# tupini07/StyleTransfer

Measured on AMD Instinct MI355X. Metric: Gatys iters/sec at 512×512 + fast_st images/sec at 256×256, 1/2/4/8 GPUs, higher is better.
Workload: dtype f32; 1 GPU; gatys_st 512x512 single image, Adam iterations (BASELINE configs[1]); one independent image per GPU (replicas); image=512, batch=1, parallelism=replicas1, graph=True

## Files before the change

### include/stx.h

```cpp
#ifndef STX_H_
#define STX_H_

#include <stddef.h>

#ifdef __cplusplus
extern "C" {
#endif

#define STX_AMAX_SLOTS 32

#define STX_OK 0
#define STX_E_INVALID 1001
#define STX_E_WORKSPACE 1002

#define STX_IN_RAW 0
#define STX_IN_RELU 1
#define STX_IN_RELU_POOL2 2
#define STX_IN_UPSAMPLE2 3
#define STX_IN_DILATE2 4

typedef struct stx_conv_params {
  const float* x;
  const float* wt;
  const float* bias;
// ... 34 lines not shown
  int unpool_out;
} stx_conv_params;

#define STX_GRAM_GROUP 8

int stx_version(void);
int stx_abi_layout(long long* out, int n);
const char* stx_last_error_string(void);
#define STX_ABI_VERSION 11
int stx_abi_version(void);

int stx_conv_weight_dims(int cin, int cout, int ks, int* cin_pad, int* cout_pad);

int stx_conv_weight_prep(const float* w, float* wt, int cout, int cin, int ks, int transpose,
                         void* stream);

size_t stx_conv_weight16_bytes(int cin, int cout, int ks, int transpose);
int stx_conv_weight_prep16(const float* w, void* wt16, float* w_amax, int cout, int cin, int ks,
                           int transpose, void* stream);
int stx_conv_weight_compose16(const float* A, int pitch, const float* a_amax, const float* w,
                              const float* w_amax, int cout, int cin, const float* scale,
                              void* wtT16, float* out_amax, void* stream);
int stx_conv_weight_prep16_pair(const float* w, void* wt16, void* wtT16, float* w_amax,
                                int cout, int cin, int ks, void* stream);
size_t stx_conv_weight16up_bytes(int cin, int cout);
int stx_conv_weight_prep16_up(const float* w, void* wt16_up, float* w_amax, int cout, int cin,
                              void* stream);
#define STX_WPREP_MAX 48
#define STX_WPREP_F32 0
#define STX_WPREP_F16 1
#define STX_WPREP_F16UP 2
typedef struct stx_wprep_job {
  const float* w;
  void* slab;
  float* w_amax;
  int kind, cout, cin, ks, transpose;
  int pad_;
} stx_wprep_job;
int stx_conv_weight_prep_batch(const stx_wprep_job* jobs, int njobs, void* stream);
int stx_amax(const float* x, long long n, float* out, void* stream);

int stx_conv_gram_tiles(const stx_conv_params* p);
int stx_conv_gram_groups(const stx_conv_params* p);

int stx_conv2d(const stx_conv_params* p, void* stream);

#define STX_WGRAD_NONE 0
#define STX_WGRAD_F32 1
#define STX_WGRAD_F16 2
#define STX_WGRAD_F16S2 3
#define STX_WGRAD_FEW16 4
typedef struct stx_wgrad_params {
  const float* x;
  const float* dy;
  float* dw;
  const float* x_amax;
  const float* dy_amax;
  void* ws;
  size_t ws_bytes;
  int accumulate;
  int n, cin, h, w, cout, ks, stride, pad, in_mode, ho, wo;
  int no_split;
} stx_wgrad_params;
int stx_conv2d_wgrad_plan(const stx_wgrad_params* p, size_t* ws_bytes);
int stx_conv2d_wgrad(const stx_wgrad_params* p, void* stream);
size_t stx_bias_grad_ws(int n, int c);
int stx_bias_grad(const float* dy, float* db, int n, int c, int hw, int accumulate,
                  void* ws, size_t ws_bytes, void* stream);

size_t stx_gram_ws(int b, int c, int hw);
int stx_gram(const float* z, float* g, int b, int c, int hw, float scale,
             const float* z_amax, void* ws, size_t ws_bytes, void* stream);

int stx_gram_coef_pitch(int c);
size_t stx_style_loss_parts(int b, int c, int hw, int* nparts);
typedef struct stx_loss_parts {
  const float* parts[8];
  int nparts[8];
  float inv[8];
  int k;
} stx_loss_parts;
int stx_loss_finalize(const stx_loss_parts* lp, float* losses, const float* extra, int m,
                      const float* w_host, float* total, void* stream);
int stx_gram_bwd(const float* coef, const float* z, float* dz, int b, int c, int h, int w,
                 const float* acc_scale_dev, const float* mask, const float* aux,
                 float aux_scale, int accumulate, void* stream);

#define STX_GUIDE_MAX 4
size_t stx_guided_style_ws(int b, int c, int hw, int R);
int stx_guided_style_loss(const float* z, const float* wts, float w_max, const float* target,
                          float* g_out, float* coef, float* loss_r, int b, int c, int hw, int R,
                          const float* lambda, float weight, const float* z_amax, void* ws,
                          size_t ws_bytes, void* stream);
int stx_guided_gram_bwd(const float* coef, const float* z, const float* wts, float* dz, int b,
                        int c, int h, int w, int R, const float* acc_scale_dev, int accumulate,
                        const float* z_amax, const float* coef_amax, void* stream);

size_t stx_color_stats_ws(int n, int h, int w);
int stx_color_stats(const float* x, double* stats, int n, int h, int w, void* ws,
                    size_t ws_bytes, void* stream);
int stx_color_affine(const float* x, const float* base, float* out, int n, int h, int w,
                     const float* M, const float* b, const float* lo, const float* hi,
                     void* stream);

size_t stx_mse_ws(long long n);
int stx_mse(const float* a, const float* b, long long n, int relu_inputs, int mode,
            float* out, float* grad, float gscale, void* ws, size_t ws_bytes, void* stream);
int stx_diff_scale(const float* a, const float* b, float* grad, long long n, float s0,
                   const float* s1_dev, const float* s2_dev, int relu, int accumulate,
                   void* stream);
#define STX_FIN_MAX 8
typedef struct stx_gram_fin_job {
  const float* parts;
  float* g_out;
  const float* target;
  float* coef;
  float* loss_parts;
  const float* mse_parts;
  float* mse_out;
  long long t_bstride;
  double mse_n;
  float scale, cA, alpha;
  int c, nsplit, b, cpad, mse_nparts;
  float* coef_amax;
} stx_gram_fin_job;
size_t stx_style_content_ws(int b, int c, int hw);
typedef struct stx_style_loss_params {
  const float* z;
  const float* parts;
  int nparts;
  const float* z_amax;
  const float* target;
  int target_batched;
  float* g_out;
  float* coef;
  float* loss;
  int b, c, hw;
  float weight, diag_alpha;
  const float* content;
  const float* mse_parts;
  float* mse_out;
  void* ws;
  size_t ws_bytes;
  stx_gram_fin_job* defer;
} stx_style_loss_params;
int stx_style_loss(const stx_style_loss_params* p, void* stream);
int stx_gram_finalize_batch(const stx_gram_fin_job* jobs, int njobs, void* stream);

int stx_loss_combine(const float* s, int k, const float* w_host, float* out, void* stream);

size_t stx_vec_ws(void);
int stx_vec_reduce(const float* a, const float* b, long long n, int op, float* out,
                   const float* mul, const float* add, float sgn, void* ws, size_t ws_bytes,
                   void* stream);
int stx_vec_axpby(float* y, const float* x, long long n, float a, const float* a_dev,
                  float a_sgn, float b, void* stream);
int stx_scalar_op(float* s, int op, int i, int j, int k, void* stream);

size_t stx_lbfgs_state_bytes(int m);
size_t stx_lbfgs_hist_bytes(long long n, int m);
size_t stx_lbfgs_ws(long long n, int m);
int stx_lbfgs_direction(float* x, const float* g, float* prev_g, float* hist, long long n, int m,
                        float lr, float tol_change, void* state, float* scal, void* ws,
                        size_t ws_bytes, void* stream);
int stx_lbfgs_grad_stats(const float* g, long long n, const float* loss, float* scal, float* clear,
                         int clear_n, void* ws, size_t ws_bytes, void* stream);

int stx_maxpool2x2_fwd(const float* x, float* y, long long* idx, int nc, int h, int w,
                       int relu_input, void* stream);
int stx_maxpool2x2_bwd(const float* dy, const long long* idx, float* dx, int nc, int h, int w,
                       void* stream);
int stx_relupool_bwd(const float* dp, const float* z, float* dz, int nc, int h, int w,
                     void* stream);
int stx_relu_fwd(const float* x, float* y, long long n, void* stream);
int stx_relu_bwd(const float* dy, const float* y, float* dx, long long n, void* stream);

size_t stx_adam_ws(void);
int stx_adam_step(float* p, const float* g, float* m, float* v, long long n, float lr,
                  float beta1, float beta2, float eps, int* step_dev, void* ws, void* stream);
int stx_adam_step_clear(float* p, const float* g, float* m, float* v, long long n, float lr,
                        float beta1, float beta2, float eps, int* step_dev, void* ws,
                        float* clear, int clear_n, void* stream);

int stx_instnorm_fwd(const float* x, const float* res, const float* gamma, const float* beta,
                     float* y, float* mean, float* rstd, int n, int c, int hw, float eps,
                     int relu, float* out_amax, void* stream);
size_t stx_instnorm_bwd_ws(int n, int c);
#define STX_PGRAD_MAX 32
typedef struct stx_in_pgrad_job {
  const float* parts;
  float* dgamma;
  float* dbeta;
  float* dbias_in;
  int n, c, accumulate, pad_;
} stx_in_pgrad_job;
int stx_instnorm_param_grads(const stx_in_pgrad_job* jobs, int njobs, void* stream);
int stx_instnorm_bwd(const float* dy, const float* beta, const float* x, const float* res,
                     const float* gamma, const float* mean, const float* rstd, float* du,
                     float* dgamma, float* dbeta, float* dbias_in, int n, int c, int hw, int relu,
                     int accumulate_params, float* out_amax, void* ws, size_t ws_bytes,
                     void* stream);

#define STX_CIN_MAX 32
typedef struct stx_cin_job {
  const float* gtab;
  const float* btab;
  float* gamma_n;
  float* beta_n;
  const float* parts;
  float* dgtab;
  float* dbtab;
  float* dbias_in;
  int c, accumulate;
} stx_cin_job;
int stx_cin_mix(const stx_cin_job* jobs, int njobs, const float* mix, int n, int S,
                void* stream);
int stx_cin_param_grads(const stx_cin_job* jobs, int njobs, const float* mix, int n, int S,
                        void* stream);

int stx_upsample2x_fwd(const float* x, float* y, int nc, int h, int w, void* stream);
int stx_upsample2x_bwd(const float* dy, float* dx, int nc, int h, int w, void* stream);

size_t stx_tv_ws(int n, int c, int h, int w);
int stx_tv_loss(const float* y, float* loss, float* grad, float gscale, const float* gscale_dev,
                int n, int c, int h, int w, float factor, void* ws, size_t ws_bytes,
                void* stream);

size_t stx_temporal_loss_ws(void);
int stx_temporal_loss(const float* y, const float* y_old, const float* x, const float* x_old,
                      long long n, float weight, float* out, void* ws, size_t ws_bytes,
                      void* stream);
int stx_temporal_loss_bwd(const float* y, const float* y_old, long long n, const float* fwd,
                          float weight, const float* g_dev, float* grad, int accumulate,
                          void* stream);

int stx_flow_compose(const float* const* prev, const float* const* fwd,
                     const float* const* bwd, int count, const float* fill, float* ref,
                     float* cmask, float* init, unsigned char* which, int n, int c, int h, int w,
                     void* stream);
int stx_flow_warp(const float* src, const float* flow, const float* fill, float* out,
                  float* valid, int n, int c, int h, int w, void* stream);
int stx_flow_consistency(const float* fwd, const float* bwd, float* cmask, int n, int h, int w,
                         void* stream);
size_t stx_masked_mse_ws(void);
int stx_masked_mse(const float* x, const float* ref, const float* mask, int n, int c, int hw,
                   float weight, float* out, float* add_to, float* grad, int accumulate,
                   void* ws, size_t ws_bytes, void* stream);

typedef struct {
  long long offset;
  int h, w;
  int top, left;
  int y0, y1;
  int resize_w, resize_h;
  int xcoef, ycoef;
  int xk, yk;
  long long tmp_offset;
} stx_image_meta;
int stx_resample_coeffs(int in_size, int out_size, int* bounds, int* kk, int kk_stride);
int stx_image_condition(const void* src, const stx_image_meta* meta, int b, int max_rows,
                        const int* coef, int size, const float* mean, const float* std_,
                        float* out, void* tmp, size_t tmp_bytes, void* stream);

#define STX_JPEG_OK 0
#define STX_JPEG_UNSUPPORTED 1
// ... 78 lines not shown
```

### styletransfer_amd/_native.py

```python
from __future__ import annotations

import ctypes as C
import os
import threading

_HERE = os.path.dirname(os.path.abspath(__file__))
LIB_PATH = os.environ.get("STX_LIB", os.path.join(_HERE, "libstx.so"))

STX_IN_RAW, STX_IN_RELU, STX_IN_RELU_POOL2, STX_IN_UPSAMPLE2, STX_IN_DILATE2 = range(5)
STX_AMAX_SLOTS = 32
STX_GRAM_GROUP = 8
STX_FLOW_JACOBI_MAXFUSE = 8
STX_ABI_VERSION = 11


def knob(name: str, default: str) -> str:
    if os.environ.get("STX_AB") != "1":
        return default
    return os.environ.get(name, default)

vp = C.c_void_p
i32 = C.c_int
i64 = C.c_longlong
f32 = C.c_float
# ... 34 lines not shown
class PGradJob(C.Structure):
    _fields_ = [("parts", vp), ("dgamma", vp), ("dbeta", vp), ("dbias_in", vp), ("n", i32),
                ("c", i32), ("accumulate", i32), ("pad_", i32)]


STX_PGRAD_MAX = 32


class CinJob(C.Structure):
    _fields_ = [("gtab", vp), ("btab", vp), ("gamma_n", vp), ("beta_n", vp), ("parts", vp),
                ("dgtab", vp), ("dbtab", vp), ("dbias_in", vp), ("c", i32), ("accumulate", i32)]


STX_CIN_MAX = 32


class LossParts(C.Structure):
    _fields_ = [("parts", vp * 8), ("nparts", i32 * 8), ("inv", f32 * 8), ("k", i32)]


class GramFinJob(C.Structure):
    _fields_ = [("parts", vp), ("g_out", vp), ("target", vp), ("coef", vp), ("loss_parts", vp),
                ("mse_parts", vp), ("mse_out", vp), ("t_bstride", i64), ("mse_n", C.c_double),
                ("scale", f32), ("cA", f32), ("alpha", f32), ("c", i32), ("nsplit", i32),
                ("b", i32), ("cpad", i32), ("mse_nparts", i32), ("coef_amax", vp)]


class StyleLossParams(C.Structure):
    _fields_ = [("z", vp), ("parts", vp), ("nparts", i32), ("z_amax", vp), ("target", vp),
                ("target_batched", i32), ("g_out", vp), ("coef", vp), ("loss", vp), ("b", i32),
                ("c", i32), ("hw", i32), ("weight", f32), ("diag_alpha", f32), ("content", vp),
                ("mse_parts", vp), ("mse_out", vp), ("ws", vp), ("ws_bytes", sz),
                ("defer", C.POINTER(GramFinJob))]


class WgradParams(C.Structure):
    _fields_ = [("x", vp), ("dy", vp), ("dw", vp), ("x_amax", vp), ("dy_amax", vp), ("ws", vp),
                ("ws_bytes", sz), ("accumulate", i32), ("n", i32), ("cin", i32), ("h", i32),
                ("w", i32), ("cout", i32), ("ks", i32), ("stride", i32), ("pad", i32),
                ("in_mode", i32), ("ho", i32), ("wo", i32), ("no_split", i32)]


class JpegDesc(C.Structure):
    _fields_ = [("status", i32), ("h", i32), ("w", i32), ("ncomp", i32), ("hs", i32 * 3),
                ("vs", i32 * 3), ("bw", i32 * 3), ("bh", i32 * 3), ("restart_interval", i32),
                ("coef_bytes", i64)]


class JpegJob(C.Structure):
    _fields_ = [("rgb_offset", i64), ("coef_offset", i64), ("qtab_offset", i64),
                ("tmp_offset", i64), ("h", i32), ("w", i32), ("ncomp", i32), ("raw", i32),
                ("hmax", i32), ("vmax", i32), ("bw", i32 * 3), ("bh", i32 * 3)]


class JpegEncJob(C.Structure):
    _fields_ = [("src_offset", i64), ("coef_offset", i64), ("qtab_offset", i64),
                ("tmp_offset", i64), ("h", i32), ("w", i32), ("ncomp", i32), ("fp32", i32),
                ("hmax", i32), ("vmax", i32), ("bw", i32 * 3), ("bh", i32 * 3),
                ("mean", f32 * 3), ("std_", f32 * 3)]


STX_JPEG_CHUNK = 32
STX_WGRAD_NONE, STX_WGRAD_F32, STX_WGRAD_F16, STX_WGRAD_F16S2, STX_WGRAD_FEW16 = range(5)
STX_FIN_MAX = 8
STX_GUIDE_MAX = 4


SIGNATURES = {
    "stx_version": (i32, []),
    "stx_abi_layout": (i32, [vp, i32]),
    "stx_last_error_string": (C.c_char_p, []),
    "stx_abi_version": (i32, []),
    "stx_conv_weight_dims": (i32, [i32, i32, i32, C.POINTER(i32), C.POINTER(i32)]),
    "stx_conv_weight_prep": (i32, [vp, vp, i32, i32, i32, i32, vp]),
    "stx_conv2d": (i32, [C.POINTER(ConvParams), vp]),
    "stx_conv_gram_tiles": (i32, [C.POINTER(ConvParams)]),
    "stx_conv_gram_groups": (i32, [C.POINTER(ConvParams)]),
    "stx_conv_weight16_bytes": (sz, [i32, i32, i32, i32]),
    "stx_conv_weight_prep16": (i32, [vp, vp, vp, i32, i32, i32, i32, vp]),
    "stx_conv_weight_prep16_pair": (i32, [vp, vp, vp, vp, i32, i32, i32, vp]),
    "stx_conv_weight16up_bytes": (sz, [i32, i32]),
    "stx_conv_weight_prep16_up": (i32, [vp, vp, vp, i32, i32, vp]),
    "stx_conv_weight_compose16": (i32, [vp, i32, vp, vp, vp, i32, i32, vp, vp, vp, vp]),
    "stx_amax": (i32, [vp, i64, vp, vp]),
    "stx_conv_weight_prep_batch": (i32, [C.POINTER(WprepJob), i32, vp]),
    "stx_conv2d_wgrad_plan": (i32, [C.POINTER(WgradParams), C.POINTER(sz)]),
    "stx_conv2d_wgrad": (i32, [C.POINTER(WgradParams), vp]),
    "stx_vec_ws": (sz, []),
    "stx_vec_reduce": (i32, [vp, vp, i64, i32, vp, vp, vp, f32, vp, sz, vp]),
    "stx_vec_axpby": (i32, [vp, vp, i64, f32, vp, f32, f32, vp]),
    "stx_scalar_op": (i32, [vp, i32, i32, i32, i32, vp]),
    "stx_lbfgs_state_bytes": (sz, [i32]),
    "stx_lbfgs_hist_bytes": (sz, [i64, i32]),
    "stx_lbfgs_ws": (sz, [i64, i32]),
    "stx_lbfgs_direction": (i32, [vp, vp, vp, vp, i64, i32, f32, f32, vp, vp, vp, sz, vp]),
    "stx_lbfgs_grad_stats": (i32, [vp, i64, vp, vp, vp, i32, vp, sz, vp]),
    "stx_bias_grad_ws": (sz, [i32, i32]),
    "stx_bias_grad": (i32, [vp, vp, i32, i32, i32, i32, vp, sz, vp]),
    "stx_gram_ws": (sz, [i32, i32, i32]),
    "stx_gram": (i32, [vp, vp, i32, i32, i32, f32, vp, vp, sz, vp]),
    "stx_gram_coef_pitch": (i32, [i32]),
    "stx_style_loss": (i32, [C.POINTER(StyleLossParams), vp]),
    "stx_style_content_ws": (sz, [i32, i32, i32]),
    "stx_gram_finalize_batch": (i32, [C.POINTER(GramFinJob), i32, vp]),
    "stx_gram_bwd": (i32, [vp, vp, vp, i32, i32, i32, i32, vp, vp, vp, f32, i32, vp]),
    "stx_guided_style_ws": (sz, [i32, i32, i32, i32]),
    "stx_guided_style_loss": (i32, [vp, vp, f32, vp, vp, vp, vp, i32, i32, i32, i32,
                                    C.POINTER(f32), f32, vp, vp, sz, vp]),
    "stx_guided_gram_bwd": (i32, [vp, vp, vp, vp, i32, i32, i32, i32, i32, vp, i32, vp, vp,
                                  vp]),
    "stx_color_stats_ws": (sz, [i32, i32, i32]),
    "stx_color_stats": (i32, [vp, vp, i32, i32, i32, vp, sz, vp]),
    "stx_color_affine": (i32, [vp, vp, vp, i32, i32, i32, C.POINTER(f32), C.POINTER(f32),
                               C.POINTER(f32), C.POINTER(f32), vp]),
    "stx_mse_ws": (sz, [i64]),
    "stx_mse": (i32, [vp, vp, i64, i32, i32, vp, vp, f32, vp, sz, vp]),
    "stx_diff_scale": (i32, [vp, vp, vp, i64, f32, vp, vp, i32, i32, vp]),
    "stx_loss_combine": (i32, [vp, i32, C.POINTER(f32), vp, vp]),
    "stx_style_loss_parts": (sz, [i32, i32, i32, C.POINTER(i32)]),
    "stx_loss_finalize": (i32, [C.POINTER(LossParts), vp, vp, i32, C.POINTER(f32), vp, vp]),
    "stx_maxpool2x2_fwd": (i32, [vp, vp, vp, i32, i32, i32, i32, vp]),
    "stx_maxpool2x2_bwd": (i32, [vp, vp, vp, i32, i32, i32, vp]),
    "stx_relupool_bwd": (i32, [vp, vp, vp, i32, i32, i32, vp]),
    "stx_relu_fwd": (i32, [vp, vp, i64, vp]),
    "stx_relu_bwd": (i32, [vp, vp, vp, i64, vp]),
    "stx_adam_ws": (sz, []),
    "stx_adam_step": (i32, [vp, vp, vp, vp, i64, f32, f32, f32, f32, vp, vp, vp]),
    "stx_adam_step_clear": (i32, [vp, vp, vp, vp, i64, f32, f32, f32, f32, vp, vp, vp, i32, vp]),
    "stx_instnorm_fwd": (i32, [vp, vp, vp, vp, vp, vp, vp, i32, i32, i32, f32, i32, vp, vp]),
    "stx_instnorm_bwd_ws": (sz, [i32, i32]),
    "stx_instnorm_param_grads": (i32, [C.POINTER(PGradJob), i32, vp]),
    "stx_instnorm_bwd": (i32, [vp, vp, vp, vp, vp, vp, vp, vp, vp, vp, vp, i32, i32, i32,
                               i32, i32, vp, vp, sz, vp]),
    "stx_cin_mix": (i32, [C.POINTER(CinJob), i32, vp, i32, i32, vp]),
    "stx_cin_param_grads": (i32, [C.POINTER(CinJob), i32, vp, i32, i32, vp]),
    "stx_upsample2x_fwd": (i32, [vp, vp, i32, i32, i32, vp]),
    "stx_upsample2x_bwd": (i32, [vp, vp, i32, i32, i32, vp]),
    "stx_tv_ws": (sz, [i32, i32, i32, i32]),
    "stx_tv_loss": (i32, [vp, vp, vp, f32, vp, i32, i32, i32, i32, f32, vp, sz, vp]),
    "stx_resample_coeffs": (i32, [i32, i32, vp, vp, i32]),
    "stx_image_condition": (i32, [vp, vp, i32, i32, vp, i32, vp, vp, vp, vp, sz, vp]),
    "stx_jpeg_info": (i32, [vp, sz, C.POINTER(JpegDesc)]),
    "stx_jpeg_entropy_decode": (i32, [vp, sz, vp, sz, vp]),
    "stx_jpeg_decode_batch": (i32, [C.POINTER(JpegJob), i32, vp, vp, vp, sz, vp]),
    "stx_jpeg_layout": (i32, [vp, i32]),
    "stx_jpeg_quant_tables": (i32, [i32, vp]),
    "stx_jpeg_encode_bound": (sz, [i32, i32, i32, i32, i32]),
    "stx_jpeg_entropy_encode": (i32, [vp, sz, i32, i32, i32, i32, i32, vp, vp, sz,
                                      C.POINTER(sz)]),
    "stx_jpeg_encode_batch": (i32, [C.POINTER(JpegEncJob), i32, vp, vp, vp, sz, vp]),
    "stx_jpeg_enc_layout": (i32, [vp, i32]),
    "stx_resample_plan": (i32, [i32, i32, i32, vp, vp, vp, i32]),
    "stx_resample2d_ws": (sz, [i32, i32, i32, i32, i32]),
    "stx_resample2d": (i32, [vp, vp, i32, i32, i32, i32, i32, vp, vp, vp, i32, vp, vp, vp, i32,
                             vp, sz, vp]),
    "stx_temporal_loss_ws": (sz, []),
    "stx_temporal_loss": (i32, [vp, vp, vp, vp, i64, f32, vp, vp, sz, vp]),
    "stx_temporal_loss_bwd": (i32, [vp, vp, i64, vp, f32, vp, vp, i32, vp]),
    "stx_flow_warp": (i32, [vp, vp, vp, vp, vp, i32, i32, i32, i32, vp]),
    "stx_flow_consistency": (i32, [vp, vp, vp, i32, i32, i32, vp]),
    "stx_flow_compose": (i32, [vp, vp, vp, i32, vp, vp, vp, vp, vp, i32, i32, i32, i32, vp]),
    "stx_masked_mse_ws": (sz, []),
    "stx_masked_mse": (i32, [vp, vp, vp, i32, i32, i32, f32, vp, vp, vp, i32, vp, sz, vp]),
    "stx_flow_pyramid": (i32, [i32, i32, i32, vp, vp, i32]),
    "stx_flow_luma": (i32, [vp, vp, i32, i32, i32, vp, vp, vp]),
    "stx_flow_linearize": (i32, [vp, vp, vp, vp, i32, i32, i32, vp]),
    "stx_flow_jacobi_ws": (sz, [i32, i32, i32]),
    "stx_flow_jacobi": (i32, [vp, vp, vp, i32, i32, i32, f32, i32, i32, vp, sz, vp]),
    "stx_flow_scale": (i32, [vp, i32, i32, i32, f32, f32, vp]),
}

_lib = None
_lock = threading.Lock()


class NativeError(RuntimeError):
    pass


def lib():
    global _lib
    if _lib is not None:
        return _lib
    with _lock:
        if _lib is None:
            if not os.path.exists(LIB_PATH):
                raise NativeError(
                    f"libstx.so not found at {LIB_PATH}; build it with "
                    f"`python -c 'import __graft_entry__ as g; g.build()'` "
                    f"(make -C styletransfer_amd/csrc)")
            try:
                L = C.CDLL(LIB_PATH)
            except OSError as e:
                raise NativeError(f"failed to load {LIB_PATH}: {e}") from e
            abi = L.stx_abi_version() if hasattr(L, "stx_abi_version") else None
            if abi != STX_ABI_VERSION:
                raise NativeError(f"{LIB_PATH}: ABI revision {abi}, this binding needs "
                                  f"{STX_ABI_VERSION} (include/stx.h STX_ABI_VERSION)")
            partial = os.environ.get("STX_LIB_PARTIAL") == "1"
            for name, (res, args) in SIGNATURES.items():
                if partial and not hasattr(L, name):
                    continue
                fn = getattr(L, name)
                fn.restype = res
                fn.argtypes = args
            _lib = L
    return _lib


def check(rc: int, what: str = ""):
    if rc != 0:
# ... 3 lines not shown
```

### styletransfer_amd/csrc/conv16.hip

```cpp
#include <stdlib.h>
#include <type_traits>

#include "common.h"
#include "conv_epi.h"
#include "wprep.h"
#include "../../include/stx.h"

namespace stx {

typedef _Float16 f16x8 __attribute__((ext_vector_type(8)));


template <int TW>
__device__ __forceinline__ void phase2_f16(f32x16 (&acc)[2][2], const stx_conv_params& p, int n,
                                           int co0, int ty0, int tx0, int wave, int h, int l32,
                                           char* smem) {
  constexpr int NPIX = 256, BM = 64;
  constexpr bool RP = TW == 64;
  const int tid = threadIdx.x;
  const size_t plane = (size_t)p.ho * p.wo;
  const float* __restrict__ A = p.p2_wt + (size_t)n * p.p2_wt_batch_stride;
  const int C2 = p.p2_c;
  const float s2 = p.p2_scale ? *p.p2_scale : 1.f;
  char* lz = smem;
  char* la = smem + 4 * NPIX * 16;
  const int q = tid & 63, cq = tid >> 6;
  const int qp = 4 * q, qrow = qp / TW, qcol = qp - qrow * TW;
  const int qy = ty0 + qrow, qx = tx0 + qcol;
  const bool vec = (p.wo & 3) == 0;
  const uint32_t zq_off = (qy < p.ho && qx < p.wo) ? (uint32_t)(qy * p.wo + qx) * 4u : BUF_OOB;
  const uint32_t pb = (uint32_t)plane * 4u;
  const float* __restrict__ z2 = p.p2_z + (size_t)n * C2 * plane;
  int bpix[2];
#pragma unroll
  for (int j = 0; j < 2; ++j) {
    int ty, tx;
    tile_pix<TW, RP>(wave, j, l32, ty, tx);
    bpix[j] = ty * TW + tx;
  }
  const int acg = tid >> 6, aco = tid & 63;
  struct Stage {
    f32x4 z[4];
    float a[8];
  };
  auto fetch = [&](int c0, Stage& g) {
    const auto rz = make_srd(z2 + (size_t)c0 * plane, (uint32_t)max(0, C2 - c0) * pb);
#pragma unroll
    for (int e = 0; e < 4; ++e) {
      const uint32_t o = zq_off + (uint32_t)(4 * cq + e) * pb;
      if (vec) {
        g.z[e] = buf_ld4(rz, o);
      } else {
#pragma unroll
        for (int k = 0; k < 4; ++k)
          g.z[e][k] = (qx + k < p.wo) ? buf_ld(rz, o + 4u * k) : 0.f;
      }
    }
    if (tid < 128) {
#pragma unroll
      for (int e = 0; e < 8; ++e) {
        const int c = c0 + acg * 8 + e, co = co0 + aco;
        g.a[e] = (c < C2 && co < p.cout_pad) ? A[(size_t)c * p.cout_pad + co] : 0.f;
      }
    }
  };
  Stage s0, s1;
  fetch(0, s0);
  if (16 < C2) fetch(16, s1);
  float m = 0.f;
  for (int base = 0; base < C2 * (BM / 4); base += 1024) {
    f32x4 v[4];
#pragma unroll
    for (int u = 0; u < 4; ++u) {
      const int idx = base + tid + 256 * u;
      const int c = idx / (BM / 4), q4 = idx - c * (BM / 4);
      const int co = co0 + 4 * q4;
      const f32x4 zero = {0.f, 0.f, 0.f, 0.f};
      v[u] = (c < C2 && co < p.cout_pad)
                 ? *reinterpret_cast<const f32x4*>(A + (size_t)c * p.cout_pad + co)
                 : zero;
    }
#pragma unroll
    for (int u = 0; u < 4; ++u)
#pragma unroll
      for (int e = 0; e < 4; ++e) m = fmaxf(m, fabsf(v[u][e]));
  }
  __shared__ float red2[4];
// ... 1306 lines not shown
    upd(v[3]);
  }
  for (long long i = 4 * n4 + t0; i < n; i += stride) upd(x[i]);
  block_max_to(out, m);
}

__device__ __forceinline__ void amax_slot_body(const float* __restrict__ x, long long n,
                                               float* __restrict__ out, int slot) {
  __shared__ float red[16];
  const long long n4 = n >> 2;
  const long long per = (n4 + STX_AMAX_SLOTS - 1) / STX_AMAX_SLOTS;
  const long long b0 = slot * per, b1 = min(n4, b0 + per);
  float m = 0.f;
  auto upd = [&](float v) {
    m = max_nan_wins(m, fabsf(v));
  };
#pragma unroll 4
  for (long long i = b0 + threadIdx.x; i < b1; i += 1024) {
    const f32x4 v = reinterpret_cast<const f32x4*>(x)[i];
    upd(v[0]);
    upd(v[1]);
    upd(v[2]);
    upd(v[3]);
  }
  if (slot == 0)
    for (long long i = 4 * n4 + threadIdx.x; i < n; i += 1024) upd(x[i]);
#pragma unroll
  for (int o = 32; o > 0; o >>= 1) {
    m = max_nan_wins(m, __shfl_xor(m, o, 64));
  }
  if ((threadIdx.x & 63) == 0) red[threadIdx.x >> 6] = m;
  __syncthreads();
  if (threadIdx.x == 0) {
    float r = red[0];
#pragma unroll
    for (int i = 1; i < 16; ++i) r = max_nan_wins(r, red[i]);
    out[slot] = r;
  }
}

__global__ void __launch_bounds__(1024) amax_slots_kernel(const float* __restrict__ x,
                                                          long long n, float* __restrict__ out) {
  amax_slot_body(x, n, out, blockIdx.x);
}

struct WprepAmax {
  const float* w[STX_WPREP_MAX];
  float* out[STX_WPREP_MAX];
  long long n[STX_WPREP_MAX];
};

__global__ void __launch_bounds__(1024) amax_batch_kernel(WprepAmax a) {
  const int j = blockIdx.x / STX_AMAX_SLOTS;
  amax_slot_body(a.w[j], a.n[j], a.out[j], blockIdx.x % STX_AMAX_SLOTS);
}

struct WprepJobs {
  stx_wprep_job job[STX_WPREP_MAX];
  int blk0[STX_WPREP_MAX + 1];
  int gin[STX_WPREP_MAX], gout[STX_WPREP_MAX];
  int njobs;
};

__global__ void __launch_bounds__(256) weight_prep_batch_kernel(WprepJobs b) {
  int j = 0;
  while (j + 1 < b.njobs && (int)blockIdx.x >= b.blk0[j + 1]) ++j;
  const stx_wprep_job& t = b.job[j];
  const int nb = b.blk0[j + 1] - b.blk0[j];
  const long long i0 = (long long)(blockIdx.x - b.blk0[j]) * 256 + threadIdx.x;
  const long long step = (long long)nb * 256;
  if (t.kind == STX_WPREP_F16)
    weight_prep16_body(t.w, reinterpret_cast<_Float16*>(t.slab), t.w_amax, t.cout, t.cin,
                       t.transpose, b.gin[j], b.gout[j], i0, step);
  else if (t.kind == STX_WPREP_F16UP)
    weight_prep16up_body(t.w, reinterpret_cast<_Float16*>(t.slab), t.w_amax, t.cout, t.cin,
                         b.gin[j] / 16, b.gout[j], i0, step);
  else
    weight_prep32_body(t.w, reinterpret_cast<float*>(t.slab), t.cout, t.cin, t.ks, t.transpose,
                       b.gin[j], b.gout[j], i0, step);
}

constexpr int WC_R = 16, WC_K = 64;

__global__ void __launch_bounds__(256)
weight_compose16_kernel(const float* __restrict__ A, int pitch, const float* __restrict__ a_amax,
                        const float* __restrict__ W, const float* __restrict__ w_amax, int C,
                        int cin, const float* __restrict__ scale, _Float16* __restrict__ slab,
                        float* __restrict__ out_amax) {
  typedef _Float16 f16x4 __attribute__((ext_vector_type(4)));
  const int K = cin * 9;
  __shared__ __attribute__((aligned(16))) float la[256][WC_R];
  __shared__ __attribute__((aligned(16))) float lw[256][WC_K];
  float (*red)[WC_R * WC_K] = reinterpret_cast<float (*)[WC_R * WC_K]>(&lw[0][0]);
  const int tid = threadIdx.x, lane = tid & 63, wave = tid >> 6;
  const int c0 = blockIdx.y * WC_R, k0 = blockIdx.x * WC_K;
  const float sc = scale ? *scale : 1.f;
  const float bound = fabsf(sc) * (float)C * read_amax(a_amax) * read_amax(w_amax);
  if (blockIdx.x == 0 && blockIdx.y == 0 && tid < STX_AMAX_SLOTS) out_amax[tid] = bound;
  const float sw = __builtin_ldexpf(1.f, 15 - amax_exp(bound));
  {
    constexpr int NLD = 256 * WC_K / 4 / 256;
    const auto ra = make_srd(A, (uint32_t)C * (uint32_t)pitch * 4u);
    const auto rw = make_srd(W, (uint32_t)C * (uint32_t)K * 4u);
    float av[WC_R];
#pragma unroll
    for (int r = 0; r < WC_R; ++r)
      av[r] = buf_ld(ra, (c0 + r < C && tid < C) ? (uint32_t)((c0 + r) * pitch + tid) * 4u : BUF_OOB);
    f32x4 v[NLD];
#pragma unroll
    for (int u = 0; u < NLD; ++u) {
      const int f = tid + 256 * u, co = f >> 4, k = k0 + 4 * (f & 15);
      v[u] = buf_ld4(rw, co < C && k < K ? (uint32_t)(co * K + k) * 4u : BUF_OOB);
    }
#pragma unroll
    for (int r = 0; r < WC_R; r += 4)
      *reinterpret_cast<f32x4*>(&la[tid][r]) = f32x4{av[r], av[r + 1], av[r + 2], av[r + 3]};
#pragma unroll
    for (int u = 0; u < NLD; ++u) {
      const int f = tid + 256 * u;
      *reinterpret_cast<f32x4*>(&lw[f >> 4][4 * (f & 15)]) = v[u];
    }
  }
  __syncthreads();
  const int r4 = 4 * (lane >> 4), q4 = 4 * (lane & 15);
  const int kk = k0 + q4;
  float acc[4][4];
#pragma unroll
  for (int a = 0; a < 4; ++a)
#pragma unroll
    for (int b = 0; b < 4; ++b) acc[a][b] = 0.f;
  const int cb = 64 * wave, ce = min(C, cb + 64);
#pragma unroll 8
  for (int co = cb; co < ce; ++co) {
    const f32x4 a4 = *reinterpret_cast<const f32x4*>(&la[co][r4]);
    const f32x4 w4 = *reinterpret_cast<const f32x4*>(&lw[co][q4]);
#pragma unroll
    for (int a = 0; a < 4; ++a)
#pragma unroll
      for (int b = 0; b < 4; ++b) acc[a][b] = fmaf(a4[a], w4[b], acc[a][b]);
  }
  __syncthreads();
  if (wave > 0) {
#pragma unroll
    for (int a = 0; a < 4; ++a)
#pragma unroll
      for (int b = 0; b < 4; ++b) red[wave - 1][(r4 + a) * WC_K + q4 + b] = acc[a][b];
  }
  __syncthreads();
  if (wave != 0) return;
  const int gout64 = rup(cin, 64);
  const int c = c0 + r4, chunk = c >> 4, cg = (c >> 3) & 1, e0 = c & 7;
#pragma unroll
  for (int b = 0; b < 4; ++b) {
    const int k = kk + b;
    if (k >= K || c >= C) continue;
    const int ci = k / 9, tap = k - 9 * ci, tapf = 8 - tap;
    f16x4 hi, lo;
#pragma unroll
    for (int a = 0; a < 4; ++a) {
      const int o = (r4 + a) * WC_K + q4 + b;
      const float v = (((acc[a][b] + red[0][o]) + red[1][o]) + red[2][o]) * sc * sw;
      hi[a] = (_Float16)v;
      lo[a] = (_Float16)(v - (float)hi[a]);
    }
    const size_t u0 = ((((size_t)chunk * 9 + tapf) * 2 + 0) * 2 + cg) * gout64 + ci;
    const size_t u1 = ((((size_t)chunk * 9 + tapf) * 2 + 1) * 2 + cg) * gout64 + ci;
    *reinterpret_cast<f16x4*>(slab + u0 * 8 + e0) = hi;
    *reinterpret_cast<f16x4*>(slab + u1 * 8 + e0) = lo;
  }
}

static int launch16_unpool(const stx_conv_params& p, hipStream_t st) {
  const int tiles_x = p.wo / 32, ntiles = tiles_x * (p.ho / 4);
  const dim3 grid(ntiles, p.cout / 64, p.n);
  const bool k2 = STX_KNOB("STX_CONV_K2", 1) != 0 && cdiv(p.cin, 16) % 2 == 0 &&
                  (long long)ntiles * (p.cout / 64) * p.n <= cus16();
  if (k2)
    hipLaunchKernelGGL((conv3x3_f16x3_v2_kernel<32, STX_IN_RAW, 4, 1, 1, true>), grid, dim3(512),
                       0, st, p, tiles_x, ntiles);
  else
    hipLaunchKernelGGL((conv3x3_f16x3_v2_kernel<32, STX_IN_RAW, 4, 1>), grid, dim3(256), 0, st, p,
                       tiles_x, ntiles);
  return check_launch("stx_conv2d(f16x3 v2 + unpool / Gram-backward epilogue)");
}

int conv2d_f16x3(const stx_conv_params& p, hipStream_t st) {
  if (p.unpool_out) return launch16_unpool(p, st);
  switch (p.stride == 2 ? LM_S2 : p.in_mode) {
    case STX_IN_RAW: return dispatch16_tw<STX_IN_RAW>(p, st);
    case STX_IN_RELU: return dispatch16_tw<STX_IN_RELU>(p, st);
    case STX_IN_RELU_POOL2: return dispatch16_tw<STX_IN_RELU_POOL2>(p, st);
    case STX_IN_UPSAMPLE2:
      if (p.wt16_up) return launch16up(p, st);
      return dispatch16_tw<STX_IN_UPSAMPLE2>(p, st);
    case LM_S2:
      if (p.pool_out || p.p2_z) {
        set_error("stx_conv2d: stride 2 takes no fused pool output / Gram phase");
        return STX_E_INVALID;
      }
      return launch16<32, LM_S2, 1>(p, st);
    default: return dispatch16_tw<STX_IN_DILATE2>(p, st);
  }
}

}

using namespace stx;

extern "C" size_t stx_conv_weight16_bytes(int cin, int cout, int ks, int transpose) {
  if (ks != 3) return 0;
  const int gin = transpose ? cout : cin, gout = transpose ? cin : cout;
  return (size_t)rup(gin, 16) * 9 * 2 * rup(gout, 64) * sizeof(_Float16);
}

extern "C" int stx_amax(const float* x, long long n, float* out, void* stream) {
  hipStream_t st = (hipStream_t)stream;
  if (!out || n < 0 || (n > 0 && !x)) {
    set_error("stx_amax: invalid arguments");
    return STX_E_INVALID;
  }
  if (reinterpret_cast<uintptr_t>(x) & 15) {
    set_error("stx_amax: x must be 16-byte aligned");
    return STX_E_INVALID;
  }
  if (n <= (8ll << 20)) {
    hipLaunchKernelGGL(amax_slots_kernel, dim3(STX_AMAX_SLOTS), dim3(1024), 0, st, x, n, out);
    return check_launch("stx_amax");
  }
  hipLaunchKernelGGL(amax_zero_kernel, dim3(1), dim3(STX_AMAX_SLOTS), 0, st, out);
  if (n == 0) return check_launch("stx_amax");
  const int blocks = (int)std::min<long long>(std::max<long long>(1, (n / 4 + 255) / 256), 512);
  hipLaunchKernelGGL(amax_kernel, dim3(blocks), dim3(256), 0, st, x, n, out);
  return check_launch("stx_amax");
}

extern "C" size_t stx_conv_weight16up_bytes(int cin, int cout) {
  if (cin <= 0 || cout <= 0) return 0;
  return (size_t)2 * rup(cin, 16) * 2 * 4 * 2 * rup(cout, 64) * sizeof(_Float16);
}

extern "C" int stx_conv_weight_prep16_up(const float* w, void* wt16_up, float* w_amax, int cout,
                                         int cin, void* stream) {
  if (!w || !wt16_up || !w_amax || cout <= 0 || cin <= 0) {
    set_error("stx_conv_weight_prep16_up: pointers non-NULL, cout / cin > 0");
    return STX_E_INVALID;
  }
  int rc = stx_amax(w, (long long)cout * cin * 9, w_amax, stream);
  if (rc) return rc;
  const long long total = (long long)rup(cin, 16) * 32 * rup(cout, 64);
  if (total >= (1ll << 31)) {
    set_error("stx_conv_weight_prep16_up: slab too large");
    return STX_E_INVALID;
// ... 38 lines not shown
  for (int j = 0; j < njobs; ++j) {
    const stx_wprep_job& t = jobs[j];
    if (!t.w || !t.slab || t.cout <= 0 || t.cin <= 0 ||
        (t.kind != STX_WPREP_F32 && t.kind != STX_WPREP_F16 && t.kind != STX_WPREP_F16UP) ||
        (t.kind != STX_WPREP_F32 && (t.ks != 3 || !t.w_amax)) ||
        (t.kind == STX_WPREP_F16UP && t.transpose)) {
      set_error("stx_conv_weight_prep_batch: job %d invalid", j);
      return STX_E_INVALID;
    }
    const int gin = t.transpose ? t.cout : t.cin, gout = t.transpose ? t.cin : t.cout;
    long long total;
    if (t.kind != STX_WPREP_F32) {
      if (reinterpret_cast<uintptr_t>(t.w) & 15) {
        set_error("stx_conv_weight_prep_batch: job %d weight not 16-byte aligned", j);
        return STX_E_INVALID;
      }
      b.gin[j] = rup(gin, 16);
      b.gout[j] = rup(gout, 64);
      total = (long long)b.gin[j] * (t.kind == STX_WPREP_F16UP ? 32 : 18) * b.gout[j];
      bool seen = false;
      for (int k = 0; k < na; ++k) {
        if (a.out[k] == t.w_amax) {
          if (a.w[k] != t.w) {
            set_error("stx_conv_weight_prep_batch: w_amax shared by two weights");
            return STX_E_INVALID;
          }
          seen = true;
        }
      }
      if (!seen) {
        a.w[na] = t.w;
        a.out[na] = t.w_amax;
        a.n[na] = (long long)t.cout * t.cin * 9;
        ++na;
      }
    } else {
      int rp, cp;
      int rc = stx_conv_weight_dims(gin, gout, t.ks, &rp, &cp);
      if (rc) return rc;
      b.gin[j] = rp * t.ks * t.ks;
      b.gout[j] = cp;
      total = (long long)b.gin[j] * cp;
    }
    if (total >= (1ll << 31)) {
      set_error("stx_conv_weight_prep_batch: job %d slab too large", j);
      return STX_E_INVALID;
    }
    b.job[j] = t;
    b.blk0[j] = blocks;
    blocks += (int)std::min<long long>((total + 4095) / 4096, 256);
  }
  b.blk0[njobs] = blocks;
  hipStream_t st = (hipStream_t)stream;
  if (na > 0)
    hipLaunchKernelGGL(amax_batch_kernel, dim3(na * STX_AMAX_SLOTS), dim3(1024), 0, st, a);
  hipLaunchKernelGGL(weight_prep_batch_kernel, dim3(blocks), dim3(256), 0, st, b);
  return check_launch("stx_conv_weight_prep_batch");
}

extern "C" int stx_conv_weight_compose16(const float* A, int pitch, const float* a_amax,
                                         const float* w, const float* w_amax, int cout, int cin,
                                         const float* scale, void* wtT16, float* out_amax,
                                         void* stream) {
  if (!A || !a_amax || !w || !w_amax || !wtT16 || !out_amax || cout <= 0 || cout > 256 ||
      cin <= 0 || cin % 4 || pitch < cout || (reinterpret_cast<uintptr_t>(w) & 15)) {
    set_error("stx_conv_weight_compose16: invalid arguments (1 <= cout <= 256, cin % 4 == 0, "
              "w 16-byte aligned)");
    return STX_E_INVALID;
  }
  const long long total = (long long)rup(cout, 16) * 9 * 2 * rup(cin, 64);
  if ((long long)cout * cin * 9 >= (1ll << 31) || total >= (1ll << 31)) {
    set_error("stx_conv_weight_compose16: weight too large");
    return STX_E_INVALID;
  }
  hipStream_t st = (hipStream_t)stream;
  if (cout % 16 || cin % 64)
    (void)hipMemsetAsync(wtT16, 0, (size_t)total * sizeof(_Float16), st);
  hipLaunchKernelGGL(weight_compose16_kernel, dim3(cdiv(cin * 9, WC_K), cdiv(cout, WC_R)), dim3(256),
                     0, st, A, pitch, a_amax, w, w_amax, cout, cin, scale,
                     reinterpret_cast<_Float16*>(wtT16), out_amax);
  return check_launch("stx_conv_weight_compose16");
}

extern "C" int stx_conv_weight_prep16(const float* w, void* wt16, float* w_amax, int cout, int cin,
                                      int ks, int transpose, void* stream) {
  if (ks != 3 || !w || !wt16 || !w_amax || cout <= 0 || cin <= 0) {
    set_error("stx_conv_weight_prep16: ks must be 3 and pointers non-NULL");
    return STX_E_INVALID;
  }
  int rc = stx_amax(w, (long long)cout * cin * 9, w_amax, stream);
  if (rc) return rc;
  const int gin = transpose ? cout : cin, gout = transpose ? cin : cout;
  const int gin16 = rup(gin, 16), gout64 = rup(gout, 64);
  const long long total = (long long)gin16 * 9 * 2 * gout64;
  if (total >= (1ll << 31)) {
    set_error("stx_conv_weight_prep16: slab too large");
    return STX_E_INVALID;
  }
  const int blocks = (int)std::min<long long>((total + 255) / 256, 4096);
  hipLaunchKernelGGL(weight_prep16_kernel, dim3(blocks), dim3(256), 0, (hipStream_t)stream, w,
                     reinterpret_cast<_Float16*>(wt16), w_amax, cout, cin, transpose, gin16,
                     gout64);
  return check_launch("stx_conv_weight_prep16");
}
```

### styletransfer_amd/csrc/elementwise.hip

```cpp
#include "common.h"
#include "../../include/stx.h"

namespace stx {

constexpr int RB = 256;
constexpr int RMAXB = 1024;

static int red_blocks(long long n) {
  return (int)std::max<long long>(1, std::min<long long>((n + RB * 8 - 1) / (RB * 8), RMAXB));
}

__global__ void __launch_bounds__(RB)
sqdiff_partial_kernel(const float* __restrict__ a, const float* __restrict__ b, long long n,
                      int relu, float* __restrict__ parts, float* __restrict__ grad,
                      float gscale) {
  __shared__ float red[RB / 64];
  float s = 0.f;
  const long long stride = (long long)gridDim.x * RB;
  for (long long i = blockIdx.x * (long long)RB + threadIdx.x; i < n; i += stride) {
    float x = a[i], y = b[i];
    if (relu) {
      x = fmaxf(x, 0.f);
      y = fmaxf(y, 0.f);
    }
    const float d = x - y;
    s += d * d;
    if (grad) grad[i] = gscale * d;
  }
  s = block_sum<RB>(s, red);
  if (threadIdx.x == 0) parts[blockIdx.x] = s;
}

__global__ void mse_finalize_kernel(const float* __restrict__ parts, int nparts, double n,
                                    int mode, float* __restrict__ out,
                                    float* __restrict__ mean_out) {
  __shared__ float red[RB / 64];
  float s = 0.f;
  for (int i = threadIdx.x; i < nparts; i += RB) s += parts[i];
  s = block_sum<RB>(s, red);
  if (threadIdx.x == 0) {
    const float mean = (float)(s / n);
    if (mode == 0) {
      *out = mean;
    } else {
      *out = (float)((double)(mean * mean) / n);
    }
    if (mean_out) *mean_out = mean;
  }
}

__global__ void __launch_bounds__(RB)
sqdiff2_partial_kernel(const float* __restrict__ a, const float* __restrict__ b, long long n,
                       float* __restrict__ parts) {
  __shared__ float red[RB / 64];
  float s = 0.f, sr = 0.f;
  const long long n4 = n / 4;
  const long long stride = (long long)gridDim.x * RB;
  for (long long i = blockIdx.x * (long long)RB + threadIdx.x; i < n4; i += stride) {
    const f32x4 x = reinterpret_cast<const f32x4*>(a)[i];
    const f32x4 y = reinterpret_cast<const f32x4*>(b)[i];
#pragma unroll
    for (int k = 0; k < 4; ++k) {
      const float d = x[k] - y[k], dr = fmaxf(x[k], 0.f) - fmaxf(y[k], 0.f);
      s += d * d;
      sr += dr * dr;
    }
  }
  for (long long i = n4 * 4 + blockIdx.x * (long long)RB + threadIdx.x; i < n; i += stride) {
    const float d = a[i] - b[i], dr = fmaxf(a[i], 0.f) - fmaxf(b[i], 0.f);
    s += d * d;
    sr += dr * dr;
  }
  s = block_sum<RB>(s, red);
  sr = block_sum<RB>(sr, red);
  if (threadIdx.x == 0) {
    parts[2 * blockIdx.x] = s;
    parts[2 * blockIdx.x + 1] = sr;
  }
}

__global__ void mse2_finalize_kernel(const float* __restrict__ parts, int nparts, double n,
                                     float* __restrict__ out) {
  __shared__ float red[RB / 64];
// ... 49 lines not shown
    const long long pl = t / ho;
    const float* src = x + pl * h * w;
    float best = -INFINITY;
    int bi = (2 * oy) * w + 2 * ox;
#pragma unroll
    for (int dy = 0; dy < 2; ++dy)
#pragma unroll
      for (int dx = 0; dx < 2; ++dx) {
        const int yy = 2 * oy + dy, xx = 2 * ox + dx;
        float v = src[yy * w + xx];
        if (relu) v = relu_keep_nan(v);
        if (v > best || isnan(v)) {
          best = v;
          bi = yy * w + xx;
        }
      }
    y[i] = best;
    if (idx) idx[i] = bi;
  }
}

__global__ void maxpool_bwd_kernel(const float* __restrict__ dy, const long long* __restrict__ idx,
                                   float* __restrict__ dx, int nc, int h, int w) {
  const int ho = h / 2, wo = w / 2;
  const long long total = (long long)nc * h * w;
  for (long long i = blockIdx.x * (long long)blockDim.x + threadIdx.x; i < total;
       i += (long long)gridDim.x * blockDim.x) {
    const int xx = (int)(i % w);
    const long long t = i / w;
    const int yy = (int)(t % h);
    const long long pl = t / h;
    const int oy = yy >> 1, ox = xx >> 1;
    float v = 0.f;
    if (oy < ho && ox < wo) {
      const long long o = (pl * ho + oy) * wo + ox;
      if (idx[o] == (long long)yy * w + xx) v = dy[o];
    }
    dx[i] = v;
  }
}

__global__ void relupool_bwd_kernel(const float* __restrict__ dp, const float* __restrict__ z,
                                    float* __restrict__ dz, int nc, int h, int w) {
  const int ho = h / 2, wo = w / 2;
  const long long total = (long long)nc * h * w;
  for (long long i = blockIdx.x * (long long)blockDim.x + threadIdx.x; i < total;
       i += (long long)gridDim.x * blockDim.x) {
    const int xx = (int)(i % w);
    const long long t = i / w;
    const int yy = (int)(t % h);
    const long long pl = t / h;
    const int oy = yy >> 1, ox = xx >> 1;
    float v = 0.f;
    const float zv = z[i];
    if (oy < ho && ox < wo && zv > 0.f) {
      const float* src = z + pl * h * w + (2 * oy) * w + 2 * ox;
      const float a0 = fmaxf(src[0], 0.f), a1 = fmaxf(src[1], 0.f);
      const float a2 = fmaxf(src[w], 0.f), a3 = fmaxf(src[w + 1], 0.f);
      int bi = 0;
      float best = a0;
      if (a1 > best) { best = a1; bi = 1; }
      if (a2 > best) { best = a2; bi = 2; }
      if (a3 > best) { best = a3; bi = 3; }
      const int me = (yy & 1) * 2 + (xx & 1);
      if (me == bi) v = dp[(pl * ho + oy) * wo + ox];
    }
    dz[i] = v;
  }
}

__global__ void relu_fwd_kernel(const float* __restrict__ x, float* __restrict__ y, long long n) {
  for (long long i = blockIdx.x * (long long)blockDim.x + threadIdx.x; i < n;
       i += (long long)gridDim.x * blockDim.x)
    y[i] = relu_keep_nan(x[i]);
}

__global__ void relu_bwd_kernel(const float* __restrict__ dy, const float* __restrict__ y,
                                float* __restrict__ dx, long long n) {
  for (long long i = blockIdx.x * (long long)blockDim.x + threadIdx.x; i < n;
       i += (long long)gridDim.x * blockDim.x)
    dx[i] = y[i] > 0.f ? dy[i] : 0.f;
}

struct AdamScalars {
  float step_size;
  float bc2_sqrt;
};

__global__ void adam_prepare_kernel(int* step, AdamScalars* sc, double lr, double b1, double b2,
                                    float* clear, int clear_n) {
  for (int i = threadIdx.x; i < clear_n; i += blockDim.x) clear[i] = 0.f;
  if (threadIdx.x) return;
  const int t = ++(*step);
  const double bc1 = 1.0 - pow(b1, (double)t);
  const double bc2 = 1.0 - pow(b2, (double)t);
  sc->step_size = (float)(lr / bc1);
  sc->bc2_sqrt = (float)sqrt(bc2);
}

__global__ void __launch_bounds__(256)
adam_kernel(float* __restrict__ p, const float* __restrict__ g, float* __restrict__ m,
            float* __restrict__ v, long long n, float b1, float b2, float eps,
            const AdamScalars* __restrict__ sc, int vec) {
  const float step_size = sc->step_size, bc2s = sc->bc2_sqrt;
  const float w1 = 1.f - b1, w2 = 1.f - b2;
  const long long n4 = vec ? n / 4 : 0;
  const long long stride = (long long)gridDim.x * blockDim.x;
  for (long long i = blockIdx.x * (long long)blockDim.x + threadIdx.x; i < n4; i += stride) {
    f32x4 pp = reinterpret_cast<f32x4*>(p)[i];
    const f32x4 gg = reinterpret_cast<const f32x4*>(g)[i];
    f32x4 mm = reinterpret_cast<f32x4*>(m)[i];
    f32x4 vv = reinterpret_cast<f32x4*>(v)[i];
#pragma unroll
    for (int k = 0; k < 4; ++k) {
      mm[k] = mm[k] + w1 * (gg[k] - mm[k]);
      vv[k] = vv[k] * b2 + w2 * gg[k] * gg[k];
      const float denom = sqrtf(vv[k]) / bc2s + eps;
      pp[k] = pp[k] + (-step_size * mm[k]) / denom;
    }
    reinterpret_cast<f32x4*>(p)[i] = pp;
    reinterpret_cast<f32x4*>(m)[i] = mm;
    reinterpret_cast<f32x4*>(v)[i] = vv;
  }
  for (long long i = n4 * 4 + blockIdx.x * (long long)blockDim.x + threadIdx.x; i < n;
       i += stride) {
    const float gg = g[i];
    const float mm = m[i] + w1 * (gg - m[i]);
    const float vv = v[i] * b2 + w2 * gg * gg;
    m[i] = mm;
    v[i] = vv;
    const float denom = sqrtf(vv) / bc2s + eps;
    p[i] = p[i] + (-step_size * mm) / denom;
  }
}

__global__ void upsample_fwd_kernel(const float* __restrict__ x, float* __restrict__ y, int nc,
                                    int h, int w) {
  const int H = 2 * h, W = 2 * w;
  const long long total = (long long)nc * H * W;
  for (long long i = blockIdx.x * (long long)blockDim.x + threadIdx.x; i < total;
       i += (long long)gridDim.x * blockDim.x) {
    const int xx = (int)(i % W);
    const long long t = i / W;
    const int yy = (int)(t % H);
    const long long pl = t / H;
    y[i] = x[(pl * h + (yy >> 1)) * w + (xx >> 1)];
  }
}

__global__ void upsample_bwd_kernel(const float* __restrict__ dy, float* __restrict__ dx, int nc,
                                    int h, int w) {
  const long long total = (long long)nc * h * w;
  const int W = 2 * w;
  for (long long i = blockIdx.x * (long long)blockDim.x + threadIdx.x; i < total;
       i += (long long)gridDim.x * blockDim.x) {
    const int xx = (int)(i % w);
    const long long t = i / w;
    const int yy = (int)(t % h);
    const long long pl = t / h;
    const float* s = dy + (pl * 2 * h + 2 * yy) * W + 2 * xx;
    dx[i] = (s[0] + s[1]) + (s[W] + s[W + 1]);
  }
}

__device__ __forceinline__ float sgn(float v) { return v > 0.f ? 1.f : (v < 0.f ? -1.f : 0.f); }

__global__ void __launch_bounds__(RB)
tv_kernel(const float* __restrict__ y, float* __restrict__ parts, float* __restrict__ grad,
          float gscale, const float* __restrict__ gscale_dev, long long total, int h, int w,
          float factor) {
  __shared__ float red[RB / 64];
  float gs = gscale * factor;
  if (gscale_dev) gs *= *gscale_dev;
  float sh = 0.f, sv = 0.f;
  const int n = (int)total;
  const uint32_t bytes = (uint32_t)n * 4u;
  const auto ry = make_srd(y, bytes);
  const auto rg = make_srd(grad ? grad : y, grad ? bytes : 0u);
  const int stride = gridDim.x * RB;
  for (int i = blockIdx.x * RB + threadIdx.x; i < n; i += stride) {
    const int q = i / w, xx = i - q * w;
    const int yy = q % h;
    const uint32_t o = (uint32_t)i * 4u;
    const float v = buf_ld(ry, o);
    const bool r_ok = xx + 1 < w, l_ok = xx > 0, d_ok = yy + 1 < h, u_ok = yy > 0;
    const float vr = buf_ld(ry, r_ok ? o + 4u : o);
    const float vl = buf_ld(ry, l_ok ? o - 4u : o);
    const float vd = buf_ld(ry, d_ok ? o + 4u * (uint32_t)w : o);
    const float vu = buf_ld(ry, u_ok ? o - 4u * (uint32_t)w : o);
    float g = 0.f;
    const float dr = v - vr, dd = v - vd;
    sh += r_ok ? fabsf(dr) : 0.f;
    g += r_ok ? sgn(dr) : 0.f;
    g -= l_ok ? sgn(vl - v) : 0.f;
    sv += d_ok ? fabsf(dd) : 0.f;
    g += d_ok ? sgn(dd) : 0.f;
    g -= u_ok ? sgn(vu - v) : 0.f;
    buf_st(rg, o, gs * g);
  }
  sh = block_sum<RB>(sh, red);
  sv = block_sum<RB>(sv, red);
  if (threadIdx.x == 0) {
    parts[2 * blockIdx.x] = sh;
    parts[2 * blockIdx.x + 1] = sv;
  }
}

__global__ void tv_finalize_kernel(const float* __restrict__ parts, int nb, float factor,
                                   float* __restrict__ out) {
  __shared__ float red[RB / 64];
  float sh = 0.f, sv = 0.f;
  for (int i = threadIdx.x; i < nb; i += RB) {
    sh += parts[2 * i];
    sv += parts[2 * i + 1];
  }
  sh = block_sum<RB>(sh, red);
// ... 103 lines not shown
  return check_launch("stx_mse");
}

extern "C" int stx_diff_scale(const float* a, const float* b, float* grad, long long n, float s0,
                              const float* s1_dev, const float* s2_dev, int relu, int accumulate,
                              void* stream) {
  hipLaunchKernelGGL(diff_scale_kernel, dim3(ew_blocks(n)), dim3(256), 0, (hipStream_t)stream, a,
                     b, grad, n, s0, s1_dev, s2_dev, relu, accumulate);
  return check_launch("stx_diff_scale");
}

extern "C" int stx_loss_combine(const float* s, int k, const float* w_host, float* out,
                                void* stream) {
  if (k < 1 || k > 16) {
    set_error("stx_loss_combine: k out of range");
    return STX_E_INVALID;
  }
  LossW w = {};
  for (int i = 0; i < k; ++i) w.w[i] = w_host[i];
  hipLaunchKernelGGL(loss_combine_kernel, dim3(1), dim3(64), 0, (hipStream_t)stream, s, k, w,
                     out);
  return check_launch("stx_loss_combine");
}

extern "C" int stx_maxpool2x2_fwd(const float* x, float* y, long long* idx, int nc, int h, int w,
                                  int relu_input, void* stream) {
  const long long n = (long long)nc * (h / 2) * (w / 2);
  if (n <= 0) {
    set_error("stx_maxpool2x2_fwd: empty");
    return STX_E_INVALID;
  }
  hipLaunchKernelGGL(maxpool_fwd_kernel, dim3(ew_blocks(n)), dim3(256), 0, (hipStream_t)stream, x,
                     y, idx, nc, h, w, relu_input);
  return check_launch("stx_maxpool2x2_fwd");
}

extern "C" int stx_maxpool2x2_bwd(const float* dy, const long long* idx, float* dx, int nc, int h,
                                  int w, void* stream) {
  const long long n = (long long)nc * h * w;
  hipLaunchKernelGGL(maxpool_bwd_kernel, dim3(ew_blocks(n)), dim3(256), 0, (hipStream_t)stream,
                     dy, idx, dx, nc, h, w);
  return check_launch("stx_maxpool2x2_bwd");
}

extern "C" int stx_relupool_bwd(const float* dp, const float* z, float* dz, int nc, int h, int w,
                                void* stream) {
  const long long n = (long long)nc * h * w;
  hipLaunchKernelGGL(relupool_bwd_kernel, dim3(ew_blocks(n)), dim3(256), 0, (hipStream_t)stream,
                     dp, z, dz, nc, h, w);
  return check_launch("stx_relupool_bwd");
}

extern "C" int stx_relu_fwd(const float* x, float* y, long long n, void* stream) {
  hipLaunchKernelGGL(relu_fwd_kernel, dim3(ew_blocks(n)), dim3(256), 0, (hipStream_t)stream, x, y,
                     n);
  return check_launch("stx_relu_fwd");
}

extern "C" int stx_relu_bwd(const float* dy, const float* y, float* dx, long long n,
                            void* stream) {
  hipLaunchKernelGGL(relu_bwd_kernel, dim3(ew_blocks(n)), dim3(256), 0, (hipStream_t)stream, dy,
                     y, dx, n);
  return check_launch("stx_relu_bwd");
}

extern "C" size_t stx_adam_ws(void) { return 64; }

extern "C" int stx_adam_step_clear(float* p, const float* g, float* m, float* v, long long n,
                                   float lr, float beta1, float beta2, float eps, int* step_dev,
                                   void* ws, float* clear, int clear_n, void* stream) {
  if (n <= 0 || !p || !g || !m || !v || !step_dev || !ws || clear_n < 0 ||
      (clear_n > 0 && !clear)) {
    set_error("stx_adam_step: invalid args");
    return STX_E_INVALID;
  }
  const int vec = (((uintptr_t)p | (uintptr_t)g | (uintptr_t)m | (uintptr_t)v) & 15) == 0;
  hipStream_t st = (hipStream_t)stream;
  AdamScalars* sc = (AdamScalars*)ws;
  hipLaunchKernelGGL(adam_prepare_kernel, dim3(1), dim3(clear_n > 0 ? 256 : 64), 0, st, step_dev,
                     sc, (double)lr, (double)beta1, (double)beta2, clear, clear_n);
  const long long units = vec ? n / 4 : n;
  const int blocks = (int)std::max<long long>(1, std::min<long long>((units + 255) / 256, 4096));
  hipLaunchKernelGGL(adam_kernel, dim3(blocks), dim3(256), 0, st, p, g, m, v, n, beta1, beta2,
                     eps, sc, vec);
  return check_launch("stx_adam_step");
}

extern "C" int stx_adam_step(float* p, const float* g, float* m, float* v, long long n, float lr,
                             float beta1, float beta2, float eps, int* step_dev, void* ws,
                             void* stream) {
  return stx_adam_step_clear(p, g, m, v, n, lr, beta1, beta2, eps, step_dev, ws, nullptr, 0,
                             stream);
}

extern "C" int stx_upsample2x_fwd(const float* x, float* y, int nc, int h, int w, void* stream) {
  const long long n = (long long)nc * 4 * h * w;
  hipLaunchKernelGGL(upsample_fwd_kernel, dim3(ew_blocks(n)), dim3(256), 0, (hipStream_t)stream,
                     x, y, nc, h, w);
  return check_launch("stx_upsample2x_fwd");
}

extern "C" int stx_upsample2x_bwd(const float* dy, float* dx, int nc, int h, int w,
                                  void* stream) {
  const long long n = (long long)nc * h * w;
  hipLaunchKernelGGL(upsample_bwd_kernel, dim3(ew_blocks(n)), dim3(256), 0, (hipStream_t)stream,
                     dy, dx, nc, h, w);
  return check_launch("stx_upsample2x_bwd");
}

extern "C" size_t stx_tv_ws(int n, int c, int h, int w) {
  return (size_t)(2 * red_blocks((long long)n * c * h * w) + 4) * sizeof(float);
}

extern "C" int stx_tv_loss(const float* y, float* loss, float* grad, float gscale,
                           const float* gscale_dev, int n, int c, int h, int w, float factor,
                           void* ws, size_t ws_bytes, void* stream) {
  const long long total = (long long)n * c * h * w;
  if (total <= 0 || !y || !loss || total >= (1ll << 29)) {
    set_error("stx_tv_loss: invalid args (or more than 2^29 elements)");
    return STX_E_INVALID;
  }
  if (!ws || ws_bytes < stx_tv_ws(n, c, h, w)) {
    set_error("stx_tv_loss: workspace too small");
    return STX_E_WORKSPACE;
  }
  hipStream_t st = (hipStream_t)stream;
  const int nb = red_blocks(total);
  hipLaunchKernelGGL(tv_kernel, dim3(nb), dim3(RB), 0, st, y, (float*)ws, grad, gscale,
                     gscale_dev, total, h, w, factor);
  hipLaunchKernelGGL(tv_finalize_kernel, dim3(1), dim3(RB), 0, st, (const float*)ws, nb, factor,
                     loss);
  return check_launch("stx_tv_loss");
}

extern "C" size_t stx_bias_grad_ws(int n, int c) { return (size_t)n * c * sizeof(float) + 64; }

static bool one_pass_bias() {
  static const bool on = STX_KNOB("STX_BIAS_ONEPASS", 1) != 0;
  return on;
}

extern "C" int stx_bias_grad(const float* dy, float* db, int n, int c, int hw, int accumulate,
                             void* ws, size_t ws_bytes, void* stream) {
  if (!ws || ws_bytes < stx_bias_grad_ws(n, c)) {
    set_error("stx_bias_grad: workspace too small");
    return STX_E_WORKSPACE;
  }
  hipStream_t st = (hipStream_t)stream;
  if ((hw & 3) == 0 && (reinterpret_cast<uintptr_t>(dy) & 15) == 0 &&
      (long long)n * hw <= 64 * 1024 && c >= 16 && one_pass_bias()) {
    hipLaunchKernelGGL(bias_grad_c_kernel, dim3(c), dim3(RB), 0, st, dy, db, n, c, hw,
                       accumulate);
    return check_launch("stx_bias_grad");
  }
  hipLaunchKernelGGL(plane_sum_kernel, dim3(n * c), dim3(RB), 0, st, dy, (float*)ws, hw);
  hipLaunchKernelGGL(sum_over_n_kernel, dim3(cdiv(c, 256)), dim3(256), 0, st, (const float*)ws,
                     db, n, c, accumulate);
  return check_launch("stx_bias_grad");
}
```

### styletransfer_amd/csrc/gram.hip

```cpp
#include "common.h"
#include "../../include/stx.h"

namespace stx {

constexpr int GT = 64;
constexpr int GKC = 64;
constexpr int GP = GKC + 1;

__device__ __forceinline__ void tile_ij(int t, int nt, int& I, int& J) {
  int i = 0;
  while (t >= nt - i) {
    t -= nt - i;
    ++i;
  }
  I = i;
  J = i + t;
}

__global__ void __launch_bounds__(256)
gram_partial_kernel(const float* __restrict__ z, float* __restrict__ ws, int c, int hw,
                    int nsplit, int split_len) {
  __shared__ __attribute__((aligned(16))) float smem[2 * GT * GP];
  float* rI = smem;
  float* rJ = smem + GT * GP;
  const int nt = cdiv(c, GT);
  const int ntu = nt * (nt + 1) / 2;
  int I, J;
  tile_ij(blockIdx.y, nt, I, J);
  const bool diag = I == J;
  const int split = blockIdx.x, b = blockIdx.z;
  const int p_begin = split * split_len;
  const int p_end = min(hw, p_begin + split_len);

  const int tid = threadIdx.x, lane = tid & 63, wave = tid >> 6;
  const int h = lane >> 5, l32 = lane & 31;
  const int qi = wave >> 1, qj = wave & 1;
  const float* zb = z + (size_t)b * c * hw;

  const int lrow = tid >> 2, lseg = (tid & 3) * 16;
  float regI[16], regJ[16];
  auto fetch = [&](int p0) {
    const int gi = I * GT + lrow, gj = J * GT + lrow;
    const float* srcI = zb + (size_t)gi * hw + p0 + lseg;
    const float* srcJ = zb + (size_t)gj * hw + p0 + lseg;
#pragma unroll
    for (int e = 0; e < 16; ++e) {
      const int pp = p0 + lseg + e;
      const bool ok = pp < p_end;
      regI[e] = (ok && gi < c) ? srcI[e] : 0.f;
      if (!diag) regJ[e] = (ok && gj < c) ? srcJ[e] : 0.f;
    }
  };
  auto store = [&]() {
#pragma unroll
    for (int e = 0; e < 16; ++e) {
      rI[lrow * GP + lseg + e] = regI[e];
      if (!diag) rJ[lrow * GP + lseg + e] = regJ[e];
    }
  };

  f32x16 acc;
#pragma unroll
  for (int r = 0; r < 16; ++r) acc[r] = 0.f;
  const float* Bsrc = diag ? rI : rJ;
  const int a_off = (qi * 32 + l32) * GP + h * 32;
  const int b_off = (qj * 32 + l32) * GP + h * 32;

  if (p_begin < p_end) fetch(p_begin);
  for (int p0 = p_begin; p0 < p_end; p0 += GKC) {
    __syncthreads();
    store();
    __syncthreads();
    if (p0 + GKC < p_end) fetch(p0 + GKC);
#pragma unroll
    for (int s = 0; s < 32; ++s)
      acc = __builtin_amdgcn_mfma_f32_32x32x2f32(rI[a_off + s], Bsrc[b_off + s], acc, 0, 0, 0);
  }
  float* out = ws + (((size_t)b * ntu + blockIdx.y) * nsplit + split) * (GT * GT);
#pragma unroll
  for (int r = 0; r < 16; ++r) {
    const int row = qi * 32 + (r & 3) + 8 * (r >> 2) + 4 * h;
    out[row * GT + qj * 32 + l32] = acc[r];
  }
// ... 487 lines not shown
      }
#pragma unroll
      for (int q = 0; q < PER; ++q) {
        if (q >= cnt) break;
        const int ob = frag_off(bj[q], st);
        fb[q][0] = *reinterpret_cast<const f16x8_t*>(base + ob);
        fb[q][1] = *reinterpret_cast<const f16x8_t*>(base + PLANE + ob);
      }
#pragma unroll
      for (int q = 0; q < PER; ++q) {
        if (q >= cnt) break;
        const int a = uA[q] ? 1 : 0;
        if (a) {
          acc[q] = __builtin_amdgcn_mfma_f32_32x32x16_f16(fa[1][0], fb[q][0], acc[q], 0, 0, 0);
          acc[q] = __builtin_amdgcn_mfma_f32_32x32x16_f16(fa[1][0], fb[q][1], acc[q], 0, 0, 0);
          acc[q] = __builtin_amdgcn_mfma_f32_32x32x16_f16(fa[1][1], fb[q][0], acc[q], 0, 0, 0);
        } else {
          acc[q] = __builtin_amdgcn_mfma_f32_32x32x16_f16(fa[0][0], fb[q][0], acc[q], 0, 0, 0);
          acc[q] = __builtin_amdgcn_mfma_f32_32x32x16_f16(fa[0][0], fb[q][1], acc[q], 0, 0, 0);
          acc[q] = __builtin_amdgcn_mfma_f32_32x32x16_f16(fa[0][1], fb[q][0], acc[q], 0, 0, 0);
        }
      }
    }
    if (c0 + T256_PX < p1) {
      stage(buf ^ 1);
      if (c0 + 2 * T256_PX < p1) fetch(c0 + 2 * T256_PX);
    }
  }
  constexpr int PITCH = 40;
  float* reg = reinterpret_cast<float*>(lds) + wave * 32 * PITCH;
  __syncthreads();
#pragma unroll
  for (int q = 0; q < PER; ++q) {
    if (q >= cnt) break;
#pragma unroll
    for (int r = 0; r < 16; ++r)
      reg[((r & 3) + 8 * (r >> 2) + 4 * h) * PITCH + l32] = acc[q][r] * inv2;
    asm volatile("s_waitcnt lgkmcnt(0)" ::: "memory");
    const int I = bi[q] >> 1, J = bj[q] >> 1, qi = bi[q] & 1, qj = bj[q] & 1;
    float* out = ws + (((size_t)b * NTU + tile_index(I, J, NT)) * nsplit + split) * (GT * GT);
#pragma unroll
    for (int k = 0; k < 4; ++k) {
      const int row = (lane >> 3) + 8 * k, c4 = lane & 7;
      const f32x4 v = *reinterpret_cast<const f32x4*>(reg + row * PITCH + 4 * c4);
      *reinterpret_cast<f32x4*>(out + (qi * 32 + row) * GT + qj * 32 + 4 * c4) = v;
      if (I == J && qi != qj) {
        f32x4 m;
#pragma unroll
        for (int e = 0; e < 4; ++e) m[e] = reg[(4 * c4 + e) * PITCH + row];
        *reinterpret_cast<f32x4*>(out + (qj * 32 + row) * GT + qi * 32 + 4 * c4) = m;
      }
    }
    asm volatile("s_waitcnt lgkmcnt(0)" ::: "memory");
  }
}

static int gram_tri256_splits(int hw, int b) {
  static const int target = std::max(8, STX_KNOB("STX_GRAM256_BLOCKS", 256));
  int want = std::max(1, target / std::max(1, b));
  want = std::min(want, std::max(1, hw / 128));
  return want;
}

static bool gram_tri256_on(int c, int hw) {
  static const bool on = STX_KNOB("STX_GRAM_TRI256", 1) != 0;
  return on && c == 256 && hw % 32 == 0;
}

static int gram_tri_splits(int c, int hw, int b) {
  static const int target = std::max(8, STX_KNOB("STX_GRAM_TRI_BLOCKS", 256));
  return std::max(1, std::min(std::max(1, target / std::max(1, b)), hw / 64));
}

static bool gram_tri_on(int c, int hw) {
  static const bool on = STX_KNOB("STX_GRAM_TRI", 1) != 0;
  return on && c == 128 && hw % 64 == 0;
}

constexpr int FEL = 64, FKL = 32, FNT = FEL / 4 * FKL;
constexpr int FSUB = GT * GT / FEL;
__host__ __device__ inline int fin_groups(int nsplit) { return nsplit <= 8 ? 4 : nsplit <= 16 ? 2 : 1; }
__host__ __device__ inline int fin_blocks_per_tile(int nsplit) { return FSUB / fin_groups(nsplit); }

template <int G>
__device__ __forceinline__ void gram_finalize_body_g(
    const float* __restrict__ ws, int c, int nsplit, float scale, float* __restrict__ g_out,
    const float* __restrict__ target, long long t_bstride, float* __restrict__ coef, int cpad,
    float cA, float alpha, float* __restrict__ loss_parts, int bx, int by, float* part,
    float* __restrict__ coef_amax) {
  constexpr int KL = FKL / G, GT_ = FNT / G;
  const int nt = cdiv(c, GT), ntu = nt * (nt + 1) / 2;
  const int tile = bx / (FSUB / G), r = threadIdx.x / GT_, sub = (bx % (FSUB / G)) * G + r;
  int I, J;
  tile_ij(tile, nt, I, J);
  const int b = by;
  const float* src = ws + ((size_t)b * ntu + tile) * nsplit * (GT * GT) + sub * FEL;
  const int t2 = threadIdx.x % GT_, q4 = t2 % (FEL / 4), kl = t2 / (FEL / 4);
  float* pr = part + (size_t)r * KL * (FEL + 1);
  {
    f32x4 s0 = {0.f, 0.f, 0.f, 0.f}, s1 = s0, s2 = s0, s3 = s0;
    const f32x4* p4 = reinterpret_cast<const f32x4*>(src) + q4;
    constexpr int ST = GT * GT / 4;
    int k = kl;
    for (; k + 3 * KL < nsplit; k += 4 * KL) {
      const f32x4 a0 = p4[(size_t)(k + 0 * KL) * ST], a1 = p4[(size_t)(k + 1 * KL) * ST];
      const f32x4 a2 = p4[(size_t)(k + 2 * KL) * ST], a3 = p4[(size_t)(k + 3 * KL) * ST];
      s0 += a0;
      s1 += a1;
      s2 += a2;
      s3 += a3;
    }
    for (; k < nsplit; k += KL) s0 += p4[(size_t)k * ST];
    const f32x4 t = (s0 + s1) + (s2 + s3);
#pragma unroll
    for (int i = 0; i < 4; ++i) pr[kl * (FEL + 1) + 4 * q4 + i] = t[i];
  }
  __syncthreads();
  float sq = 0.f, ma = 0.f;
  if (t2 < FEL) {
    const int el = t2, e = sub * FEL + el;
    float s = 0.f;
#pragma unroll 8
    for (int q = 0; q < KL; ++q) s += pr[q * (FEL + 1) + el];
    const int gi = I * GT + e / GT, gj = J * GT + e % GT;
    if (gi < c && gj < c) {
      const float g = s * scale;
      if (g_out) {
        g_out[((size_t)b * c + gi) * c + gj] = g;
        if (I != J) g_out[((size_t)b * c + gj) * c + gi] = g;
      }
      if (target) {
        const float d = g - target[(size_t)b * t_bstride + (size_t)gi * c + gj];
        sq = (I != J ? 2.f : 1.f) * d * d;
        if (coef) {
          const float a = cA * d;
          float* cb = coef + (size_t)b * cpad * cpad;
          const float ad = a + (gi == gj ? alpha : 0.f);
          cb[(size_t)gi * cpad + gj] = ad;
          if (I != J) cb[(size_t)gj * cpad + gi] = a;
          ma = fmaxf(fabsf(ad), fabsf(a));
        }
      }
    }
    if (target) {
      const float t = wave_sum(sq);
      if (t2 == 0) loss_parts[(size_t)b * ntu * FSUB + (size_t)tile * FSUB + sub] = t;
    }
    if (coef_amax) {
#pragma unroll
      for (int o = 32; o > 0; o >>= 1) ma = fmaxf(ma, __shfl_xor(ma, o, 64));
      if (t2 == 0)
        atomicMax(reinterpret_cast<unsigned int*>(coef_amax + (bx & (STX_AMAX_SLOTS - 1))),
                  __float_as_uint(ma));
    }
  }
}

__device__ __forceinline__ void gram_finalize_body(const stx_gram_fin_job& q, int bx, int by) {
  __shared__ float part[FKL * (FEL + 1)];
  __shared__ float red[FNT / 64];
  if (q.mse_out && bx == 0 && by == 0) {
    float s = 0.f, sr = 0.f;
    for (int i = threadIdx.x; i < q.mse_nparts; i += FNT) {
      s += q.mse_parts[2 * i];
      sr += q.mse_parts[2 * i + 1];
    }
    s = block_sum<FNT>(s, red);
    sr = block_sum<FNT>(sr, red);
    if (threadIdx.x == 0) {
      const float mr = (float)(sr / q.mse_n);
      q.mse_out[0] = (float)(s / q.mse_n);
      q.mse_out[1] = (float)((double)(mr * mr) / q.mse_n);
      q.mse_out[2] = mr;
    }
  }
#define STX_FIN_BODY(G)                                                                      \
  gram_finalize_body_g<G>(q.parts, q.c, q.nsplit, q.scale, q.g_out, q.target, q.t_bstride,   \
                          q.coef, q.cpad, q.cA, q.alpha, q.loss_parts, bx, by, part,         \
                          q.coef_amax)
  switch (fin_groups(q.nsplit)) {
    case 4: STX_FIN_BODY(4); break;
    case 2: STX_FIN_BODY(2); break;
    default: STX_FIN_BODY(1);
  }
#undef STX_FIN_BODY
}

__global__ void __launch_bounds__(FNT) gram_finalize_kernel(stx_gram_fin_job q) {
  gram_finalize_body(q, blockIdx.x, blockIdx.y);
}

struct FinBatch {
  stx_gram_fin_job job[STX_FIN_MAX];
  int blk0[STX_FIN_MAX + 1];
  int njobs;
};

__global__ void __launch_bounds__(FNT) gram_finalize_batch_kernel(FinBatch fb) {
  int j = 0;
  while (j + 1 < fb.njobs && (int)blockIdx.x >= fb.blk0[j + 1]) ++j;
  const stx_gram_fin_job& q = fb.job[j];
  const int local = blockIdx.x - fb.blk0[j];
  const int nt = cdiv(q.c, GT), nbx = nt * (nt + 1) / 2 * fin_blocks_per_tile(q.nsplit);
  gram_finalize_body(q, local % nbx, local / nbx);
}

__device__ __forceinline__ float wave_sum_parts(const float* __restrict__ parts, int n, int lane) {
  float s0 = 0.f, s1 = 0.f, s2 = 0.f, s3 = 0.f;
  int i = lane;
  for (; i + 192 < n; i += 256) {
    s0 += parts[i];
    s1 += parts[i + 64];
    s2 += parts[i + 128];
    s3 += parts[i + 192];
  }
  for (; i < n; i += 64) s0 += parts[i];
  return wave_sum((s0 + s1) + (s2 + s3));
}

__global__ void sum_parts_kernel(const float* __restrict__ parts, int n, float inv,
                                 float* __restrict__ out) {
  const float s = wave_sum_parts(parts, n, threadIdx.x);
  if (threadIdx.x == 0) *out = s * inv;
}

__global__ void zero_kernel(float* p, long long n) {
  for (long long i = blockIdx.x * (long long)blockDim.x + threadIdx.x; i < n;
       i += (long long)gridDim.x * blockDim.x)
    p[i] = 0.f;
}

struct LossWF {
  float w[16];
};

static void gram_geometry(int c, int hw, int b, int& nsplit, int& split_len, int& ntu) {
  const int nt = cdiv(c, GT);
  ntu = nt * (nt + 1) / 2;
  if (hw % 4 == 0) {
    int want = rup(cdiv(1024, ntu * b), 8);
    const int max_splits = std::max(1, cdiv(hw, 512));
    want = std::max(8, std::min(want, rup(max_splits, 8)));
    split_len = rup(cdiv(hw, want), 128);
    nsplit = rup(cdiv(hw, split_len), 8);
    return;
  }
  const int chunks = cdiv(hw, GKC);
  int want = cdiv(512, ntu * b);
  want = std::max(1, std::min(want, cdiv(chunks, 8)));
  const int per = cdiv(chunks, want);
  split_len = per * GKC;
  nsplit = cdiv(hw, split_len);
}

static void gram_geometry16(int c, int hw, int b, int& nsplit, int& split_len, int& ntu) {
  const int nt = cdiv(c, GT);
  ntu = nt * (nt + 1) / 2;
  static const int target = std::max(8, STX_KNOB("STX_GRAM_BLOCKS", 640));
  int want = rup(cdiv(target, ntu * b), 8);
  const int max_splits = std::max(1, cdiv(hw, 256));
  want = std::max(8, std::min(want, rup(max_splits, 8)));
  split_len = rup(cdiv(hw, want), 256);
  nsplit = rup(cdiv(hw, split_len), 8);
}

static size_t gram_parts_offset(int b, int c, int hw, int* nparts) {
  int nsplit, split_len, ntu, ns16, sl16;
  gram_geometry(c, hw, b, nsplit, split_len, ntu);
  gram_geometry16(c, hw, b, ns16, sl16, ntu);
  nsplit = std::max(nsplit, ns16);
  if (gram_tri_on(c, hw)) nsplit = std::max(nsplit, gram_tri_splits(c, hw, b));
  if (gram_tri256_on(c, hw)) nsplit = std::max(nsplit, gram_tri256_splits(hw, b));
  if (nparts) *nparts = b * ntu * FSUB;
  return (size_t)b * ntu * nsplit * GT * GT * sizeof(float);
}

static size_t gram_ws_bytes(int b, int c, int hw) {
  int nparts;
  const size_t off = gram_parts_offset(b, c, hw, &nparts);
  return off + ((size_t)nparts + 64) * sizeof(float);
}

struct MseCompanion {
  const float* content;
  float* out;
  float* parts;
  size_t parts_bytes;
};

static bool gram_partials(const float* z, int hw, const float* z_amax, void* ws, hipStream_t st,
                          stx_gram_fin_job& q, const MseCompanion* mse = nullptr) {
  const int b = q.b, c = q.c;
  const bool f16 = z_amax && hw % 8 == 0 && (reinterpret_cast<uintptr_t>(z) & 15) == 0;
  int nsplit, split_len, ntu;
  if (f16)
    gram_geometry16(c, hw, b, nsplit, split_len, ntu);
  else
    gram_geometry(c, hw, b, nsplit, split_len, ntu);
  float* slabs = (float*)ws;
  bool fused = false;
  if (f16 && gram_tri_on(c, hw)) {
    nsplit = gram_tri_splits(c, hw, b);
    split_len = rup(cdiv(hw, nsplit), 64);
    nsplit = cdiv(hw, split_len);
    if (mse && (reinterpret_cast<uintptr_t>(mse->content) & 15) == 0 &&
        mse->parts_bytes >= (size_t)2 * b * nsplit * sizeof(float)) {
      hipLaunchKernelGGL(gram_tri_f16_kernel<true>, dim3(nsplit, 1, b), dim3(256), 0, st,
                         z, slabs, hw, nsplit, split_len, z_amax, mse->content, mse->parts);
      fused = true;
      q.mse_parts = mse->parts;
      q.mse_nparts = b * nsplit;
      q.mse_out = mse->out;
    } else
      hipLaunchKernelGGL(gram_tri_f16_kernel<false>, dim3(nsplit, 1, b), dim3(256), 0, st, z, slabs,
                         hw, nsplit, split_len, z_amax);
  } else if (f16 && gram_tri256_on(c, hw)) {
    nsplit = gram_tri256_splits(hw, b);
    split_len = rup(cdiv(hw, nsplit), T256_PX);
    nsplit = cdiv(hw, split_len);
    hipLaunchKernelGGL(gram_tri256_kernel, dim3(nsplit, 1, b), dim3(512), 0, st, z, slabs, hw,
                       nsplit, split_len, z_amax);
  } else if (f16) {
    hipLaunchKernelGGL(gram_partial_f16_kernel, dim3(nsplit * ntu, 1, b), dim3(256), 0, st, z,
                       slabs, c, hw, nsplit, split_len, z_amax);
  } else if (hw % 4 == 0) {
    const int nt = cdiv(c, GT);
    hipLaunchKernelGGL(gram_partial_v2_kernel<true>, dim3(nsplit * nt, 1, b), dim3(256), 0, st,
                       z, slabs, c, hw, nsplit, split_len);
    if (ntu > nt)
      hipLaunchKernelGGL(gram_partial_v2_kernel<false>, dim3(nsplit * (ntu - nt), 1, b),
                         dim3(256), 0, st, z, slabs, c, hw, nsplit, split_len);
  } else
    hipLaunchKernelGGL(gram_partial_kernel, dim3(nsplit, ntu, b), dim3(256), 0, st, z, slabs, c,
                       hw, nsplit, split_len);
  q.parts = slabs;
  q.nsplit = nsplit;
  q.loss_parts = (float*)((char*)ws + gram_parts_offset(b, c, hw, nullptr));
  return fused;
}

static void gram_finalize(const stx_gram_fin_job& q, stx_gram_fin_job* defer, float* loss,
                          hipStream_t st) {
  if (defer) {
    *defer = q;
    return;
  }
  const int nt = cdiv(q.c, GT), ntu = nt * (nt + 1) / 2;
  hipLaunchKernelGGL(gram_finalize_kernel, dim3(ntu * fin_blocks_per_tile(q.nsplit), q.b),
                     dim3(FNT), 0, st, q);
  if (q.target && loss)
    hipLaunchKernelGGL(sum_parts_kernel, dim3(1), dim3(64), 0, st, q.loss_parts,
                       q.b * ntu * FSUB, (float)(1.0 / ((double)q.b * q.c * q.c)), loss);
}

}

using namespace stx;

extern "C" size_t stx_gram_ws(int b, int c, int hw) { return gram_ws_bytes(b, c, hw); }

extern "C" size_t stx_style_loss_parts(int b, int c, int hw, int* nparts) {
  return gram_parts_offset(b, c, hw, nparts);
}

namespace stx {
__global__ void __launch_bounds__(512) loss_finalize_kernel(stx_loss_parts lp,
                                                           float* __restrict__ losses,
                                                           const float* __restrict__ extra,
                                                           int m, LossWF w,
                                                           float* __restrict__ total) {
  __shared__ float lv[8];
  const int wave = threadIdx.x >> 6, lane = threadIdx.x & 63;
  if (wave < lp.k) {
    const float s = wave_sum_parts(lp.parts[wave], lp.nparts[wave], lane);
    if (lane == 0) lv[wave] = s * lp.inv[wave];
  }
  __syncthreads();
  if (threadIdx.x == 0) {
    float t = 0.f;
    for (int i = 0; i < lp.k; ++i) {
      losses[i] = lv[i];
      t += w.w[i] * lv[i];
    }
    for (int j = 0; j < m; ++j) t += w.w[lp.k + j] * extra[j];
    if (total) *total = t;
  }
}
}

extern "C" int stx_loss_finalize(const stx_loss_parts* lp, float* losses, const float* extra,
                                 int m, const float* w_host, float* total, void* stream) {
  if (!lp || lp->k < 0 || lp->k > 8 || m < 0 || lp->k + m > 16 || !losses ||
      (m && !extra) || (total && !w_host)) {
    set_error("stx_loss_finalize: invalid arguments");
    return STX_E_INVALID;
  }
  LossWF w{};
  for (int i = 0; i < lp->k + m && w_host; ++i) w.w[i] = w_host[i];
  hipLaunchKernelGGL(loss_finalize_kernel, dim3(1), dim3(512), 0, (hipStream_t)stream, *lp,
                     losses, extra, m, w, total);
  return check_launch("stx_loss_finalize");
}

extern "C" int stx_gram_coef_pitch(int c) { return c <= 64 ? rup(c, 64) : rup(c, 128); }

extern "C" int stx_gram(const float* z, float* g, int b, int c, int hw, float scale,
                        const float* z_amax, void* ws, size_t ws_bytes, void* stream) {
  if (b <= 0 || c <= 0 || hw <= 0 || !z) {
    set_error("gram: invalid dims");
    return STX_E_INVALID;
  }
  const size_t need = gram_ws_bytes(b, c, hw);
  if (!ws || ws_bytes < need) {
    set_error("gram: workspace %zu < %zu", ws_bytes, need);
    return STX_E_WORKSPACE;
  }
  stx_gram_fin_job q{};
  q.b = b;
  q.c = c;
  q.scale = scale;
  q.g_out = g;
  q.cpad = stx_gram_coef_pitch(c);
  gram_partials(z, hw, z_amax, ws, (hipStream_t)stream, q);
  gram_finalize(q, nullptr, nullptr, (hipStream_t)stream);
  return check_launch("gram");
}

static size_t style_content_parts_bytes(int b, int c, int hw) {
  const size_t fused = (size_t)2 * b * gram_tri_splits(c, hw, b) * sizeof(float);
  return std::max(fused, stx_mse_ws((long long)b * c * hw));
}

extern "C" size_t stx_style_content_ws(int b, int c, int hw) {
  return rup((long long)gram_ws_bytes(b, c, hw), 256) + style_content_parts_bytes(b, c, hw);
}

static int style_loss_check(const stx_style_loss_params* p) {
  const char* why = nullptr;
  if (!p || !p->target)
    why = "target is required";
  else if ((p->z != nullptr) == (p->parts != nullptr))
    why = "exactly one of z and parts is required";
  else if (p->b <= 0 || p->c <= 0 || p->hw <= 0)
    why = "invalid dims";
  else if (p->parts && (p->nparts <= 0 || (p->c > GT && p->c != 2 * GT)))
    why = "parts need nparts > 0 and c <= 64 or c == 128";
  else if (p->z ? p->mse_parts != nullptr : p->content != nullptr)
    why = "content goes with z, mse_parts with parts";
  else if ((p->content || p->mse_parts) != (p->mse_out != nullptr))
    why = "content / mse_parts and mse_out go together";
  else if (p->defer && p->loss)
    why = "a deferred finalize has no loss (stx_loss_finalize)";
  if (why) {
    set_error("stx_style_loss: %s", why);
    return STX_E_INVALID;
  }
  const size_t need = p->content ? stx_style_content_ws(p->b, p->c, p->hw)
                                 : gram_ws_bytes(p->b, p->c, p->hw);
  if (!p->ws || p->ws_bytes < need) {
    set_error("stx_style_loss: workspace %zu < %zu", p->ws_bytes, need);
    return STX_E_WORKSPACE;
  }
  return STX_OK;
}

extern "C" int stx_style_loss(const stx_style_loss_params* p, void* stream) {
  if (const int rc = style_loss_check(p)) return rc;
  hipStream_t st = (hipStream_t)stream;
  const int b = p->b, c = p->c, hw = p->hw;
  const double n = (double)c * hw;
  stx_gram_fin_job q{};
  q.b = b;
  q.c = c;
  q.cpad = stx_gram_coef_pitch(c);
  q.scale = (float)(1.0 / n);
  q.cA = (float)(p->weight * 4.0 / ((double)b * c * c * n));
  q.alpha = p->diag_alpha;
  q.g_out = p->g_out;
  q.target = p->target;
  q.t_bstride = p->target_batched ? (long long)c * c : 0;
  q.coef = p->coef;
  q.mse_n = (double)b * c * hw;
  if (p->coef && q.cpad != c) {
    const long long cnt = (long long)b * q.cpad * q.cpad;
    hipLaunchKernelGGL(zero_kernel, dim3((int)std::min<long long>((cnt + 255) / 256, 2048)),
                       dim3(256), 0, st, p->coef, cnt);
  }
  MseCompanion m{};
  if (p->content) {
    const size_t gb = rup((long long)gram_ws_bytes(b, c, hw), 256);
    m = {p->content, p->mse_out, (float*)((char*)p->ws + gb), p->ws_bytes - gb};
  }
  bool mse_pass = false;
  if (p->z) {
    const bool fused = gram_partials(p->z, hw, p->z_amax, p->ws, st, q, p->content ? &m : nullptr);
    mse_pass = p->content && !fused;
  } else {
    q.parts = p->parts;
    q.nsplit = p->nparts;
    q.loss_parts = (float*)((char*)p->ws + gram_parts_offset(b, c, hw, nullptr));
    q.mse_parts = p->mse_parts;
    q.mse_nparts = p->mse_parts ? b * p->nparts : 0;
    q.mse_out = p->mse_parts ? p->mse_out : nullptr;
  }
  gram_finalize(q, p->defer, p->loss, st);
  if (mse_pass) {
    const int rc = stx_mse(p->z, m.content, (long long)b * c * hw, 0, 2, m.out, nullptr, 1.f,
                           m.parts, m.parts_bytes, st);
    if (rc) return rc;
  }
  return check_launch("stx_style_loss");
}

extern "C" int stx_gram_finalize_batch(const stx_gram_fin_job* jobs, int njobs, void* stream) {
  if (!jobs || njobs <= 0 || njobs > STX_FIN_MAX) {
    set_error("stx_gram_finalize_batch: 1 <= njobs <= %d required", STX_FIN_MAX);
    return STX_E_INVALID;
  }
  FinBatch fb{};
  int blocks = 0;
  for (int j = 0; j < njobs; ++j) {
    const stx_gram_fin_job& q = jobs[j];
    if (!q.parts || q.c <= 0 || q.nsplit <= 0 || q.b <= 0 || !q.loss_parts) {
      set_error("stx_gram_finalize_batch: job %d invalid", j);
      return STX_E_INVALID;
    }
    const int nt = cdiv(q.c, GT);
    fb.job[j] = q;
    fb.blk0[j] = blocks;
    blocks += nt * (nt + 1) / 2 * fin_blocks_per_tile(q.nsplit) * q.b;
  }
  fb.blk0[njobs] = blocks;
  fb.njobs = njobs;
  hipLaunchKernelGGL(gram_finalize_batch_kernel, dim3(blocks), dim3(FNT), 0, (hipStream_t)stream,
                     fb);
  return check_launch("stx_gram_finalize_batch");
}

extern "C" int stx_gram_bwd(const float* coef, const float* z, float* dz, int b, int c, int h,
                            int w, const float* acc_scale_dev, const float* mask,
                            const float* aux, float aux_scale, int accumulate, void* stream) {
  stx_conv_params p = {};
  p.x = z;
  p.wt = coef;
  p.y = dz;
  p.mask = mask;
  p.aux = aux;
  p.aux_scale = aux_scale;
  p.acc_scale = acc_scale_dev;
  p.accumulate = accumulate;
  p.n = b;
  p.cin = c;
  p.h = h;
  p.w = w;
  p.cout = c;
  p.ks = 1;
  p.stride = 1;
  p.pad = 0;
  p.in_mode = STX_IN_RAW;
  p.hv = h;
  p.wv = w;
  p.ho = h;
  p.wo = w;
  stx_conv_weight_dims(c, c, 1, &p.cin_pad, &p.cout_pad);
  const int cpad = stx_gram_coef_pitch(c);
  if (p.cout_pad != cpad || p.cin_pad > cpad) {
    set_error("stx_gram_bwd: pitch mismatch");
    return STX_E_INVALID;
  }
  p.wt_batch_stride = (long long)cpad * cpad;
  return stx_conv2d(&p, stream);
}
```

### styletransfer_amd/ops.py

```python
from __future__ import annotations

import contextlib
import ctypes as C
import functools
import gc

import torch

from . import _native as N
from ._native import ConvParams, check, lib

__all__ = [
    "conv_weight_dims", "conv_weight_prep", "conv_weight_prep16", "split_eligible", "amax",
    "conv2d", "conv_out_hw", "conv2d_wgrad", "wgrad_path",
    "bias_grad", "gram", "style_loss", "gram_bwd", "guided_style_loss", "guided_gram_bwd", "mse", "diff_scale", "loss_combine",
    "maxpool2x2", "maxpool2x2_bwd", "relupool_bwd", "relu", "relu_bwd", "adam_step",
    "instnorm_fwd", "instnorm_bwd", "cin_mix", "upsample2x", "upsample2x_bwd", "tv_loss",
    "temporal_loss", "temporal_loss_bwd", "flow_warp", "flow_consistency", "flow_compose", "masked_mse",
    "color_stats", "color_affine", "resample_plan",
    "resample2d",
    "flow_pyramid", "flow_luma", "flow_linearize", "flow_jacobi", "flow_scale",
]


# ... 181 lines not shown


class CinGradBatch:

    def __init__(self):
        self.active = False
        self.jobs, self.keep, self.mix = [], [], None

    def begin(self):
        self.active = True
        self.jobs, self.keep, self.mix = [], [], None

    def add(self, parts, mix, c, dgtab, dbtab, dbias, accumulate, defer=True):
        if self.mix is not None and (self.mix.data_ptr() != mix.data_ptr() or
                                     self.mix.shape != mix.shape):
            self._launch()
        self.mix = mix
        self.keep.append(parts)
        self.jobs.append(N.CinJob(None, None, None, None, parts.data_ptr(), _p(dgtab), _p(dbtab),
                                  _p(dbias), c, int(accumulate)))
        if len(self.jobs) == N.STX_CIN_MAX or not (self.active and defer):
            self._launch()

    def _launch(self):
        if self.jobs:
            arr = (N.CinJob * len(self.jobs))(*self.jobs)
            n, S = self.mix.shape
            check(lib().stx_cin_param_grads(arr, len(self.jobs), self.mix.data_ptr(), n, S,
                                            _stream()), "stx_cin_param_grads")
        self.jobs, self.keep, self.mix = [], [], None

    def flush(self):
        self._launch()
        self.active = False


CINGRADS = CinGradBatch()


def conv_weight_dims(cin, cout, ks):
    a, b = C.c_int(), C.c_int()
    check(lib().stx_conv_weight_dims(cin, cout, ks, C.byref(a), C.byref(b)), "weight_dims")
    return a.value, b.value


def conv_weight_prep(w: torch.Tensor, transpose: bool = False) -> torch.Tensor:
    _req(w, "weight")
    cout, cin, ks, _ = w.shape
    gin, gout = (cout, cin) if transpose else (cin, cout)
    cp, op = conv_weight_dims(gin, gout, ks)
    wt = torch.empty((cp * ks * ks, op), device=w.device, dtype=torch.float32)
    check(lib().stx_conv_weight_prep(w.data_ptr(), wt.data_ptr(), cout, cin, ks, int(transpose),
                                     _stream()), "conv_weight_prep")
    return wt


def conv_weight_prep16(w: torch.Tensor, transpose: bool = False):
    _req(w, "weight")
    cout, cin, ks, _ = w.shape
    L = lib()
    nb = L.stx_conv_weight16_bytes(cin, cout, ks, int(transpose))
    if nb == 0:
        raise N.NativeError(f"no fp16-split slab for a {ks}x{ks} conv")
    wt16 = torch.empty(nb, device=w.device, dtype=torch.uint8)
    w_amax = torch.empty(N.STX_AMAX_SLOTS, device=w.device, dtype=torch.float32)
    check(L.stx_conv_weight_prep16(w.data_ptr(), wt16.data_ptr(), w_amax.data_ptr(), cout, cin,
                                   ks, int(transpose), _stream()), "conv_weight_prep16")
    return wt16, w_amax


def conv_weight_prep16_up(w: torch.Tensor):
    _req(w, "weight")
    cout, cin, ks, _ = w.shape
    assert ks == 3, ks
    L = lib()
    slab = torch.empty(L.stx_conv_weight16up_bytes(cin, cout), device=w.device, dtype=torch.uint8)
    w_amax = torch.empty(N.STX_AMAX_SLOTS, device=w.device, dtype=torch.float32)
    check(L.stx_conv_weight_prep16_up(w.data_ptr(), slab.data_ptr(), w_amax.data_ptr(), cout,
                                      cin, _stream()), "conv_weight_prep16_up")
    return slab, w_amax


def conv_weight_compose16(coef, coef_amax, w: torch.Tensor, w_amax, out_amax, scale=None,
                          out=None):
    _req(w, "weight")
    _req(coef, "coef")
    cout, cin, ks, _ = w.shape
    assert ks == 3 and coef.shape[-2] == cout and coef.numel() == cout * coef.shape[-1], coef.shape
    L = lib()
    if out is None:
        out = torch.empty(L.stx_conv_weight16_bytes(cin, cout, ks, 1), device=w.device,
                          dtype=torch.uint8)
    check(L.stx_conv_weight_compose16(coef.data_ptr(), coef.shape[-1], coef_amax.data_ptr(),
                                      w.data_ptr(), w_amax.data_ptr(), cout, cin, _p(scale),
                                      out.data_ptr(), out_amax.data_ptr(), _stream()),
          "stx_conv_weight_compose16")
    return out


def conv_weight_prep16_pair(w: torch.Tensor):
    _req(w, "weight")
    cout, cin, ks, _ = w.shape
    L = lib()
    wt16 = torch.empty(L.stx_conv_weight16_bytes(cin, cout, ks, 0), device=w.device,
                       dtype=torch.uint8)
    wtT16 = torch.empty(L.stx_conv_weight16_bytes(cin, cout, ks, 1), device=w.device,
                        dtype=torch.uint8)
    w_amax = torch.empty(N.STX_AMAX_SLOTS, device=w.device, dtype=torch.float32)
    check(L.stx_conv_weight_prep16_pair(w.data_ptr(), wt16.data_ptr(), wtT16.data_ptr(),
                                        w_amax.data_ptr(), cout, cin, ks, _stream()),
          "conv_weight_prep16_pair")
    return (wt16, w_amax), (wtT16, w_amax)


class TrainedSlabs:

    def __init__(self, convs):
        self.convs = list(convs)
        self.generation = 0
        self._retired = []
        self.slabs = None
        self._build()

    def _build(self):
        split = N.knob("STX_CONV_SPLIT", "1") != "0"
        L = lib()
        jobs = []
        if self.slabs is not None:
            self._retired.append((self.slabs, self._jobs))
            self.generation += 1
        self.slabs = []
        for conv in self.convs:
            w = conv.weight
            cout, cin, ks, _ = w.shape
            stride, pad = conv.stride[0], conv.padding[0]
            f16 = split and pad == 1 and split_eligible(cin, cout, ks, stride)
            b16 = split and pad == 1 and split_eligible(cout, cin, ks, 1)
            dev = w.device
            am = torch.empty(N.STX_AMAX_SLOTS, device=dev, dtype=torch.float32) \
                if (f16 or b16) else None
            out = []
            for t, is16 in ((0, f16), (1, b16)):
                if is16:
                    slab = torch.empty(L.stx_conv_weight16_bytes(cin, cout, ks, t), device=dev,
                                       dtype=torch.uint8)
                    jobs.append(N.WprepJob(w.data_ptr(), slab.data_ptr(), am.data_ptr(),
                                           N.STX_WPREP_F16, cout, cin, ks, t, 0))
                    out.append((None, (slab, am)))
                else:
                    gin, gout = (cout, cin) if t else (cin, cout)
                    cp, op = conv_weight_dims(gin, gout, ks)
                    slab = torch.empty((cp * ks * ks, op), device=dev, dtype=torch.float32)
                    jobs.append(N.WprepJob(w.data_ptr(), slab.data_ptr(), None,
                                           N.STX_WPREP_F32, cout, cin, ks, t, 0))
                    out.append((slab, None))
            up = None
            if f16 and stride == 1 and ks == 3 and getattr(conv, "_up_input", False) and \
                    N.knob("STX_UPAR", "1") != "0":
                up = torch.empty(L.stx_conv_weight16up_bytes(cin, cout), device=dev,
                                 dtype=torch.uint8)
                jobs.append(N.WprepJob(w.data_ptr(), up.data_ptr(), am.data_ptr(),
                                       N.STX_WPREP_F16UP, cout, cin, ks, 0, 0))
            self.slabs.append((w.data_ptr(), out[0][0], out[0][1], out[1][0], out[1][1], up))
        if len(jobs) > N.STX_WPREP_MAX:
            raise N.NativeError(f"{len(jobs)} weight slabs > STX_WPREP_MAX")
        self._jobs = (N.WprepJob * len(jobs))(*jobs)
        self._njobs = len(jobs)

    def release_retired(self):
        self._retired.clear()

    def prep(self):
        if any(c.weight.data_ptr() != s[0] for c, s in zip(self.convs, self.slabs)):
            self._build()
        if self._njobs:
            check(lib().stx_conv_weight_prep_batch(self._jobs, self._njobs, _stream()),
                  "conv_weight_prep_batch")
        for c, (_, wt, wt16, wtT, wtT16, up) in zip(self.convs, self.slabs):
            w = c.weight
# ... 245 lines not shown
    def flush(self):
        if self.jobs:
            arr = (N.GramFinJob * len(self.jobs))(*self.jobs)
            check(lib().stx_gram_finalize_batch(arr, len(self.jobs), _stream()),
                  "stx_gram_finalize_batch")
        self.jobs, self.keep = [], []


@functools.lru_cache(maxsize=None)
def _style_dims(b, c, hw, content):
    L = lib()
    npart = C.c_int()
    off = L.stx_style_loss_parts(b, c, hw, C.byref(npart))
    need = (L.stx_style_content_ws if content else L.stx_gram_ws)(b, c, hw)
    return need, off, npart.value, L.stx_gram_coef_pitch(c)


def _style_loss(b, c, hw, target, device, weight, diag_alpha, coef, defer_ws, fin, *,
                want_coef=True, loss=None, nparts=0, **source):
    _req(target, "target")
    tb = target.numel() == b * c * c and b > 1
    if not tb and target.numel() != c * c:
        raise ValueError(f"style target {tuple(target.shape)} cannot expand to ({b},{c},{c})")
    need, off, npart, cp = _style_dims(b, c, hw, source.get("content") is not None)
    if not want_coef:
        coef = None
    elif coef is None:
        coef = torch.empty((b, cp, cp), device=device, dtype=torch.float32)
    if defer_ws is not None:
        assert defer_ws.numel() >= need, (defer_ws.numel(), need)
        wp, wn = defer_ws.data_ptr(), defer_ws.numel()
    else:
        wp, wn = WS.get(need, device)
    source.update(target=target, coef=coef, loss=loss)
    p = N.StyleLossParams(target_batched=int(tb), b=b, c=c, hw=hw, weight=float(weight),
                          diag_alpha=float(diag_alpha), ws=wp, ws_bytes=wn, nparts=int(nparts),
                          **{k: t.data_ptr() for k, t in source.items() if t is not None})
    if fin is not None:
        assert defer_ws is not None
        p.defer = C.pointer(fin.new())
    check(lib().stx_style_loss(C.byref(p), _stream()), "stx_style_loss")
    if defer_ws is None:
        return loss, coef
    return (wp + off, npart, 1.0 / (b * c * c)), coef


def style_loss(z, target, weight=1.0, diag_alpha=0.0, want_coef=True, g_out=None, loss=None,
               coef=None, z_amax=None, defer_ws=None, fin=None):
    _req(z, "z")
    b, c = z.shape[:2]
    if loss is None and defer_ws is None:
        loss = torch.empty((), device=z.device, dtype=torch.float32)
    if fin is not None:
        assert g_out is None and want_coef
    return _style_loss(b, c, z[0, 0].numel(), target, z.device, weight, diag_alpha, coef,
                       defer_ws, fin, want_coef=want_coef, loss=loss, z=z, z_amax=z_amax,
                       g_out=g_out)


def style_content_loss(z, target, content, mse_out, weight=1.0, diag_alpha=0.0, coef=None,
                       z_amax=None, defer_ws=None, fin=None):
    _req(z, "z")
    _req(content, "content")
    assert content.numel() == z.numel() and mse_out.numel() >= 3
    assert defer_ws is not None
    b, c = z.shape[:2]
    return _style_loss(b, c, z[0, 0].numel(), target, z.device, weight, diag_alpha, coef,
                       defer_ws, fin, z=z, z_amax=z_amax, content=content, mse_out=mse_out)


def style_loss_from_parts(gparts, nparts, b, c, hw, target, weight=1.0, diag_alpha=0.0,
                          coef=None, defer_ws=None, fin=None, mse_parts=None, mse_out=None):
    _req(gparts, "gram partials")
    if (mse_parts is None) != (mse_out is None):
        raise ValueError("mse_parts and mse_out go together")
    if mse_parts is not None:
        _req(mse_parts, "mse_parts")
        assert mse_parts.numel() >= 2 * b * nparts and mse_out.numel() >= 3
    assert defer_ws is not None
    return _style_loss(b, c, hw, target, gparts.device, weight, diag_alpha, coef, defer_ws, fin,
                       parts=gparts, nparts=nparts, mse_parts=mse_parts, mse_out=mse_out)


def loss_finalize(parts, losses, extra=None, weights=None, total=None):
    lp = N.LossParts()
    assert len(parts) <= 8
    for i, (ptr, n, inv) in enumerate(parts):
        lp.parts[i], lp.nparts[i], lp.inv[i] = ptr, n, inv
    lp.k = len(parts)
    m = 0 if extra is None else extra.numel()
    w = None
    if weights is not None:
        w = (C.c_float * len(weights))(*[float(x) for x in weights])
    check(lib().stx_loss_finalize(C.byref(lp), losses.data_ptr(), _p(extra), m, w, _p(total),
                                  _stream()), "stx_loss_finalize")
    return losses


def gram_bwd_fused(coef, z, out=None, acc_scale=None, up_dp=None, aux=None, aux_scale=0.0,
                   out_amax=None, z_amax=None):
    b, c = z.shape[:2]
    return conv2d(z, coef, c, c, 1, pad=0, out=out, acc_scale=acc_scale, aux=aux,
                  aux_scale=aux_scale, wt_batch_stride=coef.shape[-1] * coef.shape[-2],
                  up_dp=up_dp, up_z=z if up_dp is not None else None, out_amax=out_amax,
                  in_amax=z_amax, split_1x1=z_amax is not None)


def gram_bwd(coef, z, dz=None, acc_scale=None, mask=None, aux=None, aux_scale=0.0,
             accumulate=False):
    _req(z, "z")
    b, c, h, w = z.shape
    if dz is None:
        dz = torch.empty_like(z)
    check(lib().stx_gram_bwd(coef.data_ptr(), z.data_ptr(), dz.data_ptr(), b, c, h, w,
                             _p(acc_scale), _p(mask), _p(aux), float(aux_scale), int(accumulate),
                             _stream()), "stx_gram_bwd")
    return dz


def guided_style_loss(z, wts, targets, lam, weight=1.0, z_amax=None, w_max=None, g_out=None,
                      coef=None, loss_r=None, want_coef=True, ws=None):
    _req(z, "z")
    _req(wts, "wts")
    _req(targets, "targets")
    b, c = z.shape[:2]
    hw = z[0, 0].numel()
    R = wts.shape[0]
    if wts.numel() != R * hw:
        raise ValueError(f"wts {tuple(wts.shape)} does not cover {hw} pixels per region")
    if targets.numel() != R * c * c:
        raise ValueError(f"targets {tuple(targets.shape)} is not ({R},{c},{c})")
    lam = [float(v) for v in lam]
    if len(lam) != R:
        raise ValueError(f"{len(lam)} region weights for {R} regions")
    if w_max is None:
        w_max = float(wts.max())
    if loss_r is None:
        loss_r = torch.empty(R, device=z.device, dtype=torch.float32)
    if want_coef and coef is None:
        cp = coef_pitch(c)
        coef = torch.empty((b, R, cp, cp), device=z.device, dtype=torch.float32)
    L = lib()
    need = L.stx_guided_style_ws(b, c, hw, R)
    if ws is not None:
        assert ws.numel() >= need > 0, (ws.numel(), need)
        wp, wn = ws.data_ptr(), ws.numel()
    else:
        wp, wn = WS.get(need, z.device)
    arr = (C.c_float * max(R, 1))(*lam)
    check(L.stx_guided_style_loss(z.data_ptr(), wts.data_ptr(), float(w_max), targets.data_ptr(),
                                  _p(g_out), _p(coef) if want_coef else None, loss_r.data_ptr(),
                                  b, c, hw, R, arr, float(weight), _p(z_amax), wp, wn,
                                  _stream()), "stx_guided_style_loss")
    return loss_r, (coef if want_coef else None)


def guided_gram_bwd(coef, z, wts, dz=None, acc_scale=None, accumulate=False, z_amax=None,
                    coef_amax=None):
    _req(z, "z")
    _req(wts, "wts")
    _req(coef, "coef")
    b, c, h, w = z.shape
    R = wts.shape[0]
    cp = coef_pitch(c)
    if wts.numel() != R * h * w or coef.numel() != b * R * cp * cp:
        raise ValueError(f"wts {tuple(wts.shape)} / coef {tuple(coef.shape)} do not match z "
                         f"{tuple(z.shape)} with {R} regions")
    if dz is None:
        if accumulate:
            raise ValueError("accumulate needs dz")
        dz = torch.empty_like(z)
    _req(dz, "dz")
    assert dz.shape == z.shape, (dz.shape, z.shape)
    check(lib().stx_guided_gram_bwd(coef.data_ptr(), z.data_ptr(), wts.data_ptr(), dz.data_ptr(),
                                    b, c, h, w, R, _p(acc_scale), int(accumulate), _p(z_amax),
                                    _p(coef_amax), _stream()), "stx_guided_gram_bwd")
    return dz


# ... 2 lines not shown
    _req(b, "b")
    assert a.numel() == b.numel()
    n = a.numel()
    if out is None:
        out = torch.empty({0: 1, 1: 2, 2: 3}[mode], device=a.device, dtype=torch.float32)
    L = lib()
    wp, wn = WS.get(L.stx_mse_ws(n), a.device)
    check(L.stx_mse(a.data_ptr(), b.data_ptr(), n, int(relu), mode, out.data_ptr(), _p(grad),
                    float(gscale), wp, wn, _stream()), "stx_mse")
    return out


def diff_scale(a, b, s0, s1=None, s2=None, relu=False, out=None, accumulate=False):
    if out is None:
        out = torch.empty_like(a)
    check(lib().stx_diff_scale(a.data_ptr(), b.data_ptr(), out.data_ptr(), a.numel(), float(s0),
                               _p(s1), _p(s2), int(relu), int(accumulate), _stream()),
          "stx_diff_scale")
    return out


def loss_combine(s, weights, out):
    k = len(weights)
    arr = (C.c_float * k)(*[float(x) for x in weights])
    check(lib().stx_loss_combine(s.data_ptr(), k, arr, out.data_ptr(), _stream()),
          "stx_loss_combine")
    return out


def maxpool2x2(x, relu_input=False, want_idx=True):
    _req(x, "x")
    n, c, h, w = x.shape
    y = torch.empty((n, c, h // 2, w // 2), device=x.device, dtype=torch.float32)
    idx = torch.empty(y.shape, device=x.device, dtype=torch.int64) if want_idx else None
    check(lib().stx_maxpool2x2_fwd(x.data_ptr(), y.data_ptr(), _p(idx), n * c, h, w,
                                   int(relu_input), _stream()), "stx_maxpool2x2_fwd")
    return y, idx


def maxpool2x2_bwd(dy, idx, h, w):
    n, c = dy.shape[:2]
    dx = torch.empty((n, c, h, w), device=dy.device, dtype=torch.float32)
    check(lib().stx_maxpool2x2_bwd(dy.data_ptr(), idx.data_ptr(), dx.data_ptr(), n * c, h, w,
                                   _stream()), "stx_maxpool2x2_bwd")
    return dx


def relupool_bwd(dp, z, out=None):
    n, c, h, w = z.shape
    if out is None:
        out = torch.empty_like(z)
    check(lib().stx_relupool_bwd(dp.data_ptr(), z.data_ptr(), out.data_ptr(), n * c, h, w,
                                 _stream()), "stx_relupool_bwd")
    return out


def relu(x):
    _req(x, "x")
    y = torch.empty_like(x)
    check(lib().stx_relu_fwd(x.data_ptr(), y.data_ptr(), x.numel(), _stream()), "stx_relu_fwd")
    return y


def relu_bwd(dy, y):
    dx = torch.empty_like(dy)
    check(lib().stx_relu_bwd(dy.data_ptr(), y.data_ptr(), dx.data_ptr(), dy.numel(), _stream()),
          "stx_relu_bwd")
    return dx


def adam_step(p, g, m, v, step_dev, ws, lr=1e-3, beta1=0.9, beta2=0.999, eps=1e-8,
              clear=None):
    if clear is not None:
        _req(clear, "clear")
        check(lib().stx_adam_step_clear(p.data_ptr(), g.data_ptr(), m.data_ptr(), v.data_ptr(),
                                        p.numel(), float(lr), float(beta1), float(beta2),
                                        float(eps), step_dev.data_ptr(), ws.data_ptr(),
                                        clear.data_ptr(), clear.numel(), _stream()),
              "stx_adam_step_clear")
        return
    check(lib().stx_adam_step(p.data_ptr(), g.data_ptr(), m.data_ptr(), v.data_ptr(), p.numel(),
                              float(lr), float(beta1), float(beta2), float(eps),
                              step_dev.data_ptr(), ws.data_ptr(), _stream()), "stx_adam_step")


def _mix_of(mix, n):
    _req(mix, "mix")
    if mix.dim() != 2 or mix.shape[0] != n:
        raise ValueError(f"mix {tuple(mix.shape)}: [{n}][S] expected")
    return mix


def cin_mix(tables, mix):
    tables = list(tables)
    if not tables:
        return []
    n, S = _mix_of(mix, mix.shape[0]).shape
    jobs, out = [], []
    buf = torch.empty(2 * n * sum(g.shape[1] for g, _ in tables), device=mix.device,
                      dtype=torch.float32)
    o = 0
    for g, b in tables:
        _req(g, "gtab")
        _req(b, "btab")
        c = g.shape[1]
        if tuple(g.shape) != (S, c) or tuple(b.shape) != (S, c):
            raise ValueError(f"style tables {tuple(g.shape)} / {tuple(b.shape)}: [{S}][c] expected")
        gn, bn = buf[o:o + n * c].view(n, c), buf[o + n * c:o + 2 * n * c].view(n, c)
        o += 2 * n * c
        out.append((gn, bn))
        jobs.append(N.CinJob(g.data_ptr(), b.data_ptr(), gn.data_ptr(), bn.data_ptr(), None, None,
                             None, None, c, 0))
    for i in range(0, len(jobs), N.STX_CIN_MAX):
        chunk = jobs[i:i + N.STX_CIN_MAX]
        check(lib().stx_cin_mix((N.CinJob * len(chunk))(*chunk), len(chunk), mix.data_ptr(), n, S,
                                _stream()), "stx_cin_mix")
    return out


def instnorm_fwd(x, gamma, beta, res=None, eps=1e-5, relu=False, out=None, out_amax=None,
                 per_sample=False):
    _req(x, "x")
    n, c = x.shape[:2]
    hw = x[0, 0].numel()
    if per_sample:
        for t in (gamma, beta):
            if t is None or tuple(_req(t, "per-sample affine").shape) != (n, c):
                raise ValueError(f"per_sample: gamma and beta must be [{n}][{c}]")
        n, c = 1, n * c
    if out is None:
        out = torch.empty_like(x)
    mean = torch.empty(n * c, device=x.device, dtype=torch.float32)
    rstd = torch.empty_like(mean)
    check(lib().stx_instnorm_fwd(x.data_ptr(), _p(res), _p(gamma), _p(beta), out.data_ptr(),
                                 mean.data_ptr(), rstd.data_ptr(), n, c, hw, float(eps),
                                 int(relu), _p(out_amax), _stream()), "stx_instnorm_fwd")
    return out, mean, rstd


def instnorm_bwd(dy, beta, x, res, gamma, mean, rstd, relu=False, dgamma=None, dbeta=None,
                 accumulate=False, out_amax=None, dbias_in=None, per_sample=False, mix=None):
    n, c = x.shape[:2]
    hw = x[0, 0].numel()
    du = torch.empty_like(x)
    L = lib()
    need = L.stx_instnorm_bwd_ws(n, c)
    if per_sample:
        if gamma is None or tuple(gamma.shape) != (n, c) or beta is None or \
                tuple(beta.shape) != (n, c):
            raise ValueError(f"per_sample: gamma and beta must be [{n}][{c}]")
        want = dgamma is not None or dbeta is not None or dbias_in is not None
        if want:
            S = _mix_of(mix, n).shape[1]
            for t in (dgamma, dbeta):
                if t is not None and tuple(_req(t, "table gradient").shape) != (S, c):
                    raise ValueError(f"per_sample: table gradients must be [{S}][{c}]")
            parts = torch.empty(need, device=x.device, dtype=torch.uint8)
            wp, wn = parts.data_ptr(), need
        else:
            wp, wn = WS.get(need, x.device)
        check(L.stx_instnorm_bwd(dy.data_ptr(), beta.data_ptr(), x.data_ptr(), _p(res),
                                 gamma.data_ptr(), mean.data_ptr(), rstd.data_ptr(),
                                 du.data_ptr(), None, None, None, 1, n * c, hw, int(relu), 0,
                                 _p(out_amax), wp, wn, _stream()), "stx_instnorm_bwd")
        if want:
            CINGRADS.add(parts, mix, c, dgamma, dbeta, dbias_in, accumulate,
# ... 363 lines not shown
```

### styletransfer_amd/vgg.py

```python
from __future__ import annotations

import os
from dataclasses import dataclass, field

import numpy as np
import torch

from . import _native as N
from . import ops
from . import weights as W

STYLE_CONVS = (0, 1, 2, 3, 4)
CONTENT_CONV = 3
N_LOSSES = 7
VGG_CONV_SHAPES = [(64, 3), (64, 64), (128, 64), (128, 128), (256, 128)]
IN_MODES = [N.STX_IN_RAW, N.STX_IN_RELU, N.STX_IN_RELU_POOL2, N.STX_IN_RELU,
            N.STX_IN_RELU_POOL2]


def load_vgg19_weights(path: str | None = None, seed: int = 1234):
    path = path or os.environ.get("STX_VGG19_WEIGHTS")
    if path and os.path.exists(path):
        sd = torch.load(path, map_location="cpu", weights_only=True)
        out = []
# ... 45 lines not shown

    def fuses_pool(self, l, wo):
        return (l + 1 < len(IN_MODES) and IN_MODES[l + 1] == N.STX_IN_RELU_POOL2
                and self.wt16[l] is not None and self.wt16[l + 1] is not None and wo > 32)

    def gram_tiles(self, l, ho, wo, n=1):
        cout, cin = VGG_CONV_SHAPES[l]
        if (cin >= 16 and self.wt16[l] is None) or N.knob("STX_GRAM_FUSE", "1") == "0":
            return 0
        return ops.conv_gram_tiles(cin, cout, ho, wo, n=n, in_mode=self._run_mode(l, wo))

    def _run_mode(self, l, wo):
        mode = IN_MODES[l]
        if mode == N.STX_IN_RELU_POOL2 and l > 0 and self.fuses_pool(l - 1, 2 * wo):
            return N.STX_IN_RAW
        return mode

    def gram_groups(self, l, ho, wo, n=1):
        if N.knob("STX_GRAM_GROUPED", "0") != "1" or not self.gram_tiles(l, ho, wo, n):
            return 0
        cout, cin = VGG_CONV_SHAPES[l]
        return ops.conv_gram_groups(cin, cout, ho, wo, n=n, in_mode=self._run_mode(l, wo))

    def forward(self, x, upto=5, outs=None, amax=None, pools=None, on_layer=None, grams=None,
                content=None, keep=None):
        zs, cur, pin = [], x, None
        for l in range(upto):
            cout, cin = VGG_CONV_SHAPES[l]
            src, mode = cur, IN_MODES[l]
            if mode == N.STX_IN_RELU_POOL2 and pin is not None:
                src, mode = pin, N.STX_IN_RAW
            kw = {}
            if amax is not None:
                kw = dict(in_amax=slot(amax, l) if l > 0 else None,
                          out_amax=slot(amax, l + 1))
            pin = None
            if l + 1 < upto and self.fuses_pool(l, src.shape[3]):
                shp = (src.shape[0], cout, src.shape[2] // 2, src.shape[3] // 2)
                pin = pools[l] if pools is not None and pools[l] is not None else \
                    torch.empty(shp, device=src.device, dtype=torch.float32)
                if pools is not None:
                    pools[l] = pin
                kw["pool_out"] = pin
                if keep is not None and l not in keep and outs is None and grams is None \
                        and on_layer is None and self.wt16[l] is not None:
                    kw["pool_only"] = True
            if grams is not None and grams[l] is not None:
                if isinstance(grams[l], tuple):
                    kw["gram_part"], kw["gram_cnt"] = grams[l]
                else:
                    kw["gram_part"] = grams[l]
                if content is not None and l == CONTENT_CONV:
                    kw["mse_ref"], kw["mse_parts"] = content
            cur = ops.conv2d(src, self.wt[l], cin, cout, 3, in_mode=mode, bias=self.b[l],
                             out=None if outs is None else outs[l], wt16=self.wt16[l], **kw)
            zs.append(cur)
            if on_layer is not None:
                on_layer(l, cur)
        return zs

    def style_targets(self, style_image):
        zs = self.forward(style_image.contiguous())
        return [ops.gram(z) for z in zs]


@dataclass
class LossState:
    z: list = field(default_factory=list)
    coef: list = field(default_factory=list)
    c4: torch.Tensor = None
    losses: torch.Tensor = None
    fmean: torch.Tensor = None
    folded: bool = False
    alpha: float = 0.0
    amax: torch.Tensor = None
    amax_cleared: bool = False
    coef_amax: list = None
    pools: list = field(default_factory=lambda: [None] * 5)
    lws: list = field(default_factory=lambda: [None] * 5)
    parts: list = field(default_factory=lambda: [None] * 5)
    grams: list = field(default_factory=lambda: [None] * 5)
    fin_jobs: list = None
    mse_parts: torch.Tensor = None


def tap_weights(style_weight, layer_weights=None):
    if not isinstance(style_weight, (int, float)):
        if layer_weights is not None:
            raise ValueError("style_weight per tap and layer_weights: give one of them")
        sws = [float(v) for v in style_weight]
        if len(sws) != 5:
            raise ValueError(f"style weights: one float or five, got {len(sws)}")
        return sws
    if layer_weights is None:
        return [float(style_weight)] * 5
    lw = [float(v) for v in layer_weights]
    if len(lw) != 5 or min(lw) < 0 or not all(np.isfinite(lw)):
        raise ValueError(f"style_layer_weights: five non-negative numbers expected, got {lw}")
    return [float(style_weight) * v for v in lw]


def _folded_style(style_weight, layer_weights):
    if layer_weights is None:
        return float(style_weight)
    return tap_weights(float(style_weight), layer_weights)


def loss_forward(feat: VGGFeatures, targets, x, c4, st: LossState | None = None,
                 folded_weights=None, total=None, extra_slot=False):
    if st is None:
        st = LossState()
    dev = x.device
    if st.amax is None:
        st.amax = torch.zeros(LOSS_AMAX_GROUPS * N.STX_AMAX_SLOTS, device=dev,
                              dtype=torch.float32)
    elif not st.amax_cleared:
        st.amax.zero_()
    st.amax_cleared = False
    if st.losses is None:
        st.losses = torch.empty(N_LOSSES + 1, device=dev, dtype=torch.float32)
        st.fmean = st.losses[6:8]
    if not st.coef:
        st.coef = [None] * 5
    B, _, H, W = x.shape
    z4_shape = (B, 128, H // 2, W // 2)
    assert tuple(c4.shape) == z4_shape, (c4.shape, z4_shape)
    sws, alpha = [1.0] * 5, 0.0
    st.folded = folded_weights is not None
    if st.folded:
        sws = tap_weights(folded_weights[0])
        alpha = float(folded_weights[1]) * 2.0 / (B * 128 * (H // 2) * (W // 2))
    st.alpha = alpha
    st.c4 = c4
    split = N.knob("STX_GRAM_SPLIT", "1") != "0"

    hs = [H, H, H // 2, H // 2, H // 4]
    for l in range(5):
        nt = feat.gram_tiles(l, hs[l], hs[l] * W // H, n=B) if split else 0
        ng = feat.gram_groups(l, hs[l], hs[l] * W // H, n=B) if nt else 0
        if nt == 0:
            st.grams[l] = None
        elif ng:
            if not isinstance(st.grams[l], tuple) or st.grams[l][0].numel() != B * (nt + ng) * 4096:
                st.grams[l] = (torch.empty(B * (nt + ng) * 4096, device=dev, dtype=torch.float32),
                               torch.zeros(B * ng, device=dev, dtype=torch.int32))
        elif st.grams[l] is None or isinstance(st.grams[l], tuple) or \
                st.grams[l].numel() != B * ops.gram_tile_units(VGG_CONV_SHAPES[l][0]) * nt * 4096:
            st.grams[l] = torch.empty(B * ops.gram_tile_units(VGG_CONV_SHAPES[l][0]) * nt * 4096,
                                      device=dev, dtype=torch.float32)

    fuse_content = N.knob("STX_CONTENT_FUSE", "1") != "0"
    content = None
    if st.grams[CONTENT_CONV] is not None and fuse_content:
        nt4 = feat.gram_tiles(CONTENT_CONV, hs[CONTENT_CONV], hs[CONTENT_CONV] * W // H, n=B)
        if st.mse_parts is None or st.mse_parts.numel() != 2 * B * nt4:
            st.mse_parts = torch.empty(2 * B * nt4, device=dev, dtype=torch.float32)
        content = (c4, st.mse_parts)
    fin = ops.FinalizeBatch() if N.knob("STX_FIN_BATCH", "1") != "0" else None

    def tap_loss(i, l, z, b_, c_, fuse_mse):
        if fuse_mse:
            st.parts[i], st.coef[i] = ops.style_content_loss(
                z, targets[i], c4, st.losses[5:8], weight=sws[i], diag_alpha=alpha,
                coef=st.coef[i], z_amax=slot(st.amax, l + 1), defer_ws=st.lws[i], fin=fin)
            return
        fused_mse = False
        if st.grams[l] is not None:
            gp = st.grams[l]
            if isinstance(gp, tuple):
                ng = gp[1].numel() // b_
                gp = gp[0][gp[0].numel() - b_ * ng * 4096:]
            fused_mse = l == CONTENT_CONV and content is not None
            st.parts[i], st.coef[i] = ops.style_loss_from_parts(
                gp, gp.numel() // (b_ * ops.gram_tile_units(c_) * 4096), b_, c_, z[0, 0].numel(),
                targets[i], weight=sws[i], diag_alpha=alpha if l == CONTENT_CONV else 0.0,
                coef=st.coef[i], defer_ws=st.lws[i], fin=fin,
                mse_parts=st.mse_parts if fused_mse else None,
                mse_out=st.losses[5:8] if fused_mse else None)
        else:
            st.parts[i], st.coef[i] = ops.style_loss(
                z, targets[i], weight=sws[i], diag_alpha=alpha if l == CONTENT_CONV else 0.0,
                coef=st.coef[i], z_amax=slot(st.amax, l + 1) if split else None,
                defer_ws=st.lws[i], fin=fin)
        if l == CONTENT_CONV and not fused_mse:
            ops.mse(z, c4, mode=2, out=st.losses[5:8])

    st.coef_amax = [None] * 5

    def on_layer(l, z):
        i = STYLE_CONVS.index(l)
        b_, c_ = z.shape[:2]
        fuse_mse = l == CONTENT_CONV and st.grams[l] is None and split and fuse_content
        L = N.lib()
        need = (L.stx_style_content_ws if fuse_mse else L.stx_gram_ws)(b_, c_, z[0, 0].numel())
        if st.lws[i] is None or st.lws[i].numel() < need:
            st.lws[i] = torch.empty(need, device=dev, dtype=torch.uint8)
        njobs = len(fin.jobs) if fin is not None else 0
        tap_loss(i, l, z, b_, c_, fuse_mse)
        if i in COEF_AMAX_SLOT and fin is not None and len(fin.jobs) == njobs + 1:
            st.coef_amax[i] = slot(st.amax, COEF_AMAX_SLOT[i])
            fin.jobs[-1].coef_amax = st.coef_amax[i].data_ptr()

    st.z = feat.forward(x, 5, st.z if st.z else None, amax=st.amax, pools=st.pools,
                        on_layer=on_layer, grams=st.grams, content=content)
    if fin is not None:
        st.fin_jobs = list(fin.jobs)
        fin.flush()
    w = None
    extra = None
    if total is not None:
        fw = folded_weights if folded_weights is not None else (1.0, 1.0)
        w = tap_weights(fw[0]) + [float(fw[1])]
        extra = st.losses[5:6]
        if extra_slot:
            w += [0.0, 0.0, 1.0]
            extra = st.losses[5:9]
    ops.loss_finalize(st.parts, st.losses[0:5], extra=extra, weights=w, total=total)
    return st


LOSS_AMAX_GROUPS = 17
COEF_AMAX_SLOT = {0: 11, 1: 15, 2: 12, 3: 16, 4: 14}
COMPOSE_AMAX_SLOT = 13


def slot(amax, k):
    return amax[k * N.STX_AMAX_SLOTS:(k + 1) * N.STX_AMAX_SLOTS]


def loss_values(st: LossState):
    return st.losses[:N_LOSSES]


def loss_backward(feat: VGGFeatures, st: LossState, g=None, dx=None, feature_grad=True,
                  scratch=None):
    z = st.z
    B = z[0].shape[0]
    sc = scratch if scratch is not None else {}

    def buf(name, shape):
        t = sc.get(name)
        if t is None or tuple(t.shape) != tuple(shape):
            t = torch.empty(shape, device=z[0].device, dtype=torch.float32)
            sc[name] = t
        return t

    folded = st.folded
    s = (lambda i: None) if folded else (lambda i: g[i:i + 1])
    am = st.amax
    sp = feat.wt16[1] is not None
    n4 = (B, 128, z[3].shape[2] // 2, z[3].shape[3] // 2)
    ca = st.coef_amax if st.coef_amax else [None] * 5
    dz4 = None
    up4 = None
    if sp and ca[3] is not None and n4[3] % 32 == 0 and n4[2] % 4 == 0 and \
            N.knob("STX_UNPOOL_FUSE", "1") != "0":
        up4 = dict(unpool_out=(z[3], st.coef[3], ca[3], slot(am, 4), s(3)),
                   aux=st.c4 if folded else None, aux_scale=-st.alpha,
                   out_amax=slot(am, 7) if folded else None)
    if sp and B == 1 and feat.wtT16[4] is not None and ca[4] is not None and \
            N.knob("STX_COMPOSE", "1") != "0":
        sc["compose5"] = ops.conv_weight_compose16(
            st.coef[4], ca[4], feat.w[4], feat.wtT16[4][1], slot(am, COMPOSE_AMAX_SLOT),
            scale=s(4), out=sc.get("compose5"))
        cout, cin = VGG_CONV_SHAPES[4]
        if up4:
            dz4 = ops.conv2d(z[4], None, cout, cin, 3, out=buf("dz4", z[3].shape),
                             wt16=(sc["compose5"], slot(am, COMPOSE_AMAX_SLOT)),
                             in_amax=slot(am, 5), **up4)
        else:
            dp2 = ops.conv2d(z[4], None, cout, cin, 3, out=buf("dp2", n4),
                             wt16=(sc["compose5"], slot(am, COMPOSE_AMAX_SLOT)),
                             in_amax=slot(am, 5))
    else:
        dz5 = ops.gram_bwd_fused(st.coef[4], z[4], out=buf("dz5", z[4].shape), acc_scale=s(4),
                                 out_amax=slot(am, 6), z_amax=slot(am, 5) if sp else None)
        if up4:
            dz4 = feat.dgrad(4, dz5, buf("dz4", z[3].shape), in_amax=slot(am, 6), **up4)
        else:
            dp2 = feat.dgrad(4, dz5, buf("dp2", n4), in_amax=slot(am, 6))
    if dz4 is None:
        dz4 = ops.gram_bwd_fused(st.coef[3], z[3], out=buf("dz4", z[3].shape), acc_scale=s(3),
                                 up_dp=dp2, aux=st.c4 if folded else None, aux_scale=-st.alpha,
                                 out_amax=slot(am, 7) if folded else None,
                                 z_amax=slot(am, 4) if sp else None)
    n = z[3].numel()
    dz4_amax = slot(am, 7) if folded else None
    if not folded:
        ops.diff_scale(z[3], st.c4, 2.0 / n, s1=g[5:6], out=dz4, accumulate=True)
        if feature_grad:
            ops.diff_scale(z[3], st.c4, 4.0 / (float(n) * float(n)), s1=g[6:7],
                           s2=st.fmean[1:2], relu=True, out=dz4, accumulate=True)
    dz3 = feat.dgrad(3, dz4, buf("dz3", z[2].shape), mask=z[2], p2_z=z[2],
                     p2_coef=st.coef[2], p2_scale=s(2), in_amax=dz4_amax, out_amax=slot(am, 8),
                     p2_amax=slot(am, 3), p2_wt_amax=ca[2])
    n2 = (B, 64, z[1].shape[2] // 2, z[1].shape[3] // 2)
    if sp and ca[1] is not None and n2[3] % 32 == 0 and n2[2] % 4 == 0 and \
            N.knob("STX_UNPOOL_FUSE", "1") != "0":
        dz2 = feat.dgrad(2, dz3, buf("dz2", z[1].shape), in_amax=slot(am, 8),
                         out_amax=slot(am, 9),
                         unpool_out=(z[1], st.coef[1], ca[1], slot(am, 2), s(1)))
    else:
        dp1 = feat.dgrad(2, dz3, buf("dp1", n2), in_amax=slot(am, 8))
        dz2 = ops.gram_bwd_fused(st.coef[1], z[1], out=buf("dz2", z[1].shape), acc_scale=s(1),
                                 up_dp=dp1, out_amax=slot(am, 9),
                                 z_amax=slot(am, 2) if sp else None)
    dz1 = feat.dgrad(1, dz2, buf("dz1", z[0].shape), mask=z[0], p2_z=z[0],
                     p2_coef=st.coef[0], p2_scale=s(0), in_amax=slot(am, 9), p2_amax=slot(am, 1),
                     out_amax=slot(am, 10) if sp else None, p2_wt_amax=ca[0])
    xs = (B, 3, z[0].shape[2], z[0].shape[3])
    if dx is None:
        dx = torch.empty(xs, device=z[0].device, dtype=torch.float32)
    return feat.dgrad(0, dz1, dx, in_amax=slot(am, 10) if sp else None)


def content_target(feat: VGGFeatures, content, out=None, amax=None):
    return feat.forward(content.contiguous(), 4, amax=amax, keep={3})[3] if out is None else \
        feat.forward(content.contiguous(), 4, [None, None, None, out], amax=amax)[3]


def _own_temporal(eng, temporal):
    eng.temporal = eng.tloss = None
    if temporal is None:
        return
    ref, mask, weight = temporal
    x = eng.x
    if ref.numel() != x.numel() or mask.numel() != x.numel() // x.shape[1]:
        raise ValueError(f"temporal: ref {tuple(ref.shape)} / mask {tuple(mask.shape)} do not "
                         f"match the canvas {tuple(x.shape)}")
    ref = ref.to(x.device, torch.float32).reshape(x.shape).clone().contiguous()
    mask = mask.to(x.device, torch.float32).reshape(x.shape[0], *x.shape[2:]).clone().contiguous()
    eng.temporal = (ref, mask, float(weight))
    eng.tloss = torch.zeros(1, device=x.device, dtype=torch.float32)


def _temporal_term(eng):
    ref, mask, weight = eng.temporal
    ops.masked_mse(eng.x, ref, mask, weight, out=eng.tloss, add_to=eng.total, grad=eng.grad,
                   accumulate=True)


class GatysEngine:

    def __init__(self, feat: VGGFeatures, style_image, content_image, style_weight=100_000,
                 content_weight=1, lr=1e-3, betas=(0.9, 0.999), eps=1e-8, init=None,
                 targets=None, style_layer_weights=None, temporal=None):
        dev = feat.device
        self.feat = feat
        if targets is None:
            targets = feat.style_targets(style_image.to(dev, torch.float32))
        self.targets = [t.reshape(t.shape[-2:]).contiguous() for t in targets]
        self.content = content_image.to(dev, torch.float32).contiguous()
        self.c4 = content_target(feat, self.content).clone()
        src = self.content if init is None else init.to(dev, torch.float32)
        self.x = src.clone().contiguous()
        _own_temporal(self, temporal)
        self.grad = torch.zeros_like(self.x)
        self.m = torch.zeros_like(self.x)
        self.v = torch.zeros_like(self.x)
        self.step_dev = torch.zeros(1, dtype=torch.int32, device=dev)
        self.adam_ws = torch.zeros(16, dtype=torch.float32, device=dev)
        self.lr, self.betas, self.eps = lr, betas, eps
        self.sw, self.cw = _folded_style(style_weight, style_layer_weights), float(content_weight)
        self.g = torch.tensor(tap_weights(self.sw) + [self.cw, 0.0], device=dev,
                              dtype=torch.float32)
        self.total = torch.zeros((), device=dev, dtype=torch.float32)
        self.st = LossState()
        self.scratch = {}
        self.graph = None

    def _iteration(self):
        loss_forward(self.feat, self.targets, self.x, self.c4, self.st,
                     folded_weights=(self.sw, self.cw), total=self.total)
        loss_backward(self.feat, self.st, dx=self.grad, feature_grad=False,
                      scratch=self.scratch)
        if self.temporal is not None:
            _temporal_term(self)
        ops.adam_step(self.x, self.grad, self.m, self.v, self.step_dev, self.adam_ws, self.lr,
                      self.betas[0], self.betas[1], self.eps, clear=self.st.amax)
        self.st.amax_cleared = True

    def retarget(self, content, init=None, temporal_ref=None, temporal_mask=None):
        content = content.to(self.x.device, torch.float32).contiguous()
        if content.shape != self.content.shape:
            raise ValueError(f"retarget: content {tuple(content.shape)}, the engine holds "
                             f"{tuple(self.content.shape)}")
        if self.temporal is None and (temporal_ref is not None or temporal_mask is not None):
            raise ValueError("retarget: the engine was built without a temporal term")
        self.content = content
        content_target(self.feat, self.content, out=self.c4)
        if temporal_ref is not None:
            self.temporal[0].copy_(temporal_ref.reshape(self.x.shape))
        if temporal_mask is not None:
            self.temporal[1].copy_(temporal_mask.reshape(self.temporal[1].shape))
        self.x.copy_(self.content if init is None else init.reshape(self.x.shape))
        self.m.zero_()
        self.v.zero_()
        self.step_dev.zero_()
        return self

    def capture(self, warmup=2):
        s = torch.cuda.Stream()
        s.wait_stream(torch.cuda.current_stream())
        with torch.cuda.stream(s):
            for _ in range(warmup):
                self._iteration()
        torch.cuda.current_stream().wait_stream(s)
        self.graph = torch.cuda.CUDAGraph()
        with ops.graph_capture(self.graph):
            self._iteration()
        return self

    def step(self):
        if self.graph is not None:
            self.graph.replay()
        else:
            self._iteration()
        return self.total

    def run(self, steps, graph=True):
        if steps <= 0:
            return self.x
        if not graph:
            for _ in range(steps):
                self._iteration()
            return self.x
        self.capture(warmup=1)
        for _ in range(steps - 1):
            self.graph.replay()
        return self.x

    def losses(self):
        return loss_values(self.st)


class GatysLBFGS:

    def __init__(self, feat: VGGFeatures, style_image, content_image, style_weight=100_000,
                 content_weight=1, targets=None, init=None, style_layer_weights=None,
                 temporal=None, **lbfgs_kw):
        from .optim import LBFGS
        dev = feat.device
        self.feat = feat
        if targets is None:
            targets = feat.style_targets(style_image.to(dev, torch.float32))
        self.targets = [t.reshape(t.shape[-2:]).contiguous() for t in targets]
        self.content = content_image.to(dev, torch.float32).contiguous()
        self.c4 = content_target(feat, self.content).clone()
        src = self.content if init is None else init.to(dev, torch.float32)
        self.x = src.clone().contiguous()
        _own_temporal(self, temporal)
        self.grad = torch.zeros_like(self.x)
        self.sw, self.cw = _folded_style(style_weight, style_layer_weights), float(content_weight)
        self.total = torch.zeros((), device=dev, dtype=torch.float32)
        self.st = LossState()
        self.scratch = {}
        self.opt = LBFGS([self.x], **lbfgs_kw)
        self.opt._buffers(self.x.numel(), dev)
        self.g_eval = self.g_iter = None
        self._at_x = None
        self.closure_runs = 0

    def _closure(self):
        loss_forward(self.feat, self.targets, self.x, self.c4, self.st,
                     folded_weights=(self.sw, self.cw), total=self.total)
        loss_backward(self.feat, self.st, dx=self.grad, feature_grad=False,
                      scratch=self.scratch)
        if self.temporal is not None:
            _temporal_term(self)
        self.opt.grad_stats(self.grad.view(-1), self.total.view(1), clear=self.st.amax)
        self.st.amax_cleared = True

    def capture(self):
        s = torch.cuda.Stream()
        s.wait_stream(torch.cuda.current_stream())
        with torch.cuda.stream(s):
            self._closure()
        torch.cuda.current_stream().wait_stream(s)
        b = self.opt._buf
        self.g_eval = torch.cuda.CUDAGraph()
        with ops.graph_capture(self.g_eval):
            self._closure()
            b["host"].copy_(b["scal"], non_blocking=True)
        self.g_iter = torch.cuda.CUDAGraph()
        with ops.graph_capture(self.g_iter, pool=self.g_eval.pool()):
            self.opt.direction(self.grad.view(-1))
            self._closure()
            b["host"].copy_(b["scal"], non_blocking=True)
        return self

    def _read(self):
        loss, gmax, gtd, t, smax, flag = self.opt._scal_host(0, 1, 3, 4, 5, 6)
        return loss, gmax, gtd, t, smax, flag

    def step(self, on_eval=None):
        if self.g_iter is None:
            self.capture()

        def evaluate():
            self.g_eval.replay()
            self.closure_runs += 1
            loss, gmax = self.opt._scal_host(0, 1)
            self._at_x = (loss, loss, gmax, self.grad.view(-1))
            return self._at_x

        pending = []

        def move(g):
            self.g_iter.replay()
            self.closure_runs += 1
            loss, gmax, gtd, t, smax, flag = self._read()
            self._at_x = (loss, loss, gmax, self.grad.view(-1))
            pending.append(self._at_x)
            return gtd, t, smax, bool(flag)

        def evaluate_after_move():
            return pending.pop() if pending else evaluate()

        first, self._at_x = self._at_x, None
        ret = self.opt.run(evaluate_after_move, move, first=first, on_eval=on_eval)
        if self._at_x is None:
            self._at_x = first
        return ret

    @property
    def func_evals(self):
        return self.opt.state[self.x].get("func_evals", 0)

    def history(self):
        pairs, n_iter = self.opt._scal(8, 9)
        return int(pairs), int(n_iter)

    def run(self, steps):
        for _ in range(steps):
            self.step()
        return self.x


TAP_POOLS = (0, 0, 1, 1, 2)


def guides_for_taps(mask_hw):
    m = torch.as_tensor(mask_hw).detach().to("cpu", torch.float64)
    single = m.dim() == 2
    if single:
        m = m[None]
    if m.dim() != 3:
        raise ValueError(f"guide must be [H][W] or [R][H][W], got {tuple(m.shape)}")
# ... 194 lines not shown
```

Baseline: 1590 iters/s.

## Fold loss finalize and Adam prepare into the weight-compose kernel as rider blocks

Two small serial kernels, the loss finalize and the Adam bias-correction prepare, become extra rider blocks of the conv5 weight-compose kernel launch. The amax clear moves into the last block of the Adam update kernel, so the per-iteration launch chain gets shorter. The gram finalize reduction also gains a deeper unrolled path for large split counts. The cost is more coupling between unrelated stages, plus the ordering assumption that the deferred loss and prepare finish before their consumers on the stream.

Measured after the change: 1612 iters/s (median of 6 runs). +1.4%, better.

```diff
diff --git a/include/stx.h b/include/stx.h
--- a/include/stx.h
+++ b/include/stx.h
@@ -140,6 +140,12 @@
 } stx_loss_parts;
 int stx_loss_finalize(const stx_loss_parts* lp, float* losses, const float* extra, int m,
                       const float* w_host, float* total, void* stream);
+int stx_conv_weight_compose16_tail(const float* A, int pitch, const float* a_amax, const float* w,
+                                   const float* w_amax, int cout, int cin, const float* scale,
+                                   void* wtT16, float* out_amax, const stx_loss_parts* lp,
+                                   float* losses, const float* extra, int m, const float* w_host,
+                                   float* total, int* step_dev, void* adam_ws, float lr,
+                                   float beta1, float beta2, void* stream);
 int stx_gram_bwd(const float* coef, const float* z, float* dz, int b, int c, int h, int w,
                  const float* acc_scale_dev, const float* mask, const float* aux,
                  float aux_scale, int accumulate, void* stream);
@@ -239,6 +245,9 @@
 int stx_adam_step_clear(float* p, const float* g, float* m, float* v, long long n, float lr,
                         float beta1, float beta2, float eps, int* step_dev, void* ws,
                         float* clear, int clear_n, void* stream);
+int stx_adam_step_prepared(float* p, const float* g, float* m, float* v, long long n, float beta1,
+                           float beta2, float eps, const void* ws, float* clear, int clear_n,
+                           void* stream);
 
 int stx_instnorm_fwd(const float* x, const float* res, const float* gamma, const float* beta,
                      float* y, float* mean, float* rstd, int n, int c, int hw, float eps,
diff --git a/styletransfer_amd/_native.py b/styletransfer_amd/_native.py
--- a/styletransfer_amd/_native.py
+++ b/styletransfer_amd/_native.py
@@ -140,6 +140,9 @@
     "stx_conv_weight16up_bytes": (sz, [i32, i32]),
     "stx_conv_weight_prep16_up": (i32, [vp, vp, vp, i32, i32, vp]),
     "stx_conv_weight_compose16": (i32, [vp, i32, vp, vp, vp, i32, i32, vp, vp, vp, vp]),
+    "stx_conv_weight_compose16_tail": (i32, [vp, i32, vp, vp, vp, i32, i32, vp, vp, vp,
+                                             C.POINTER(LossParts), vp, vp, i32,
+                                             C.POINTER(f32), vp, vp, vp, f32, f32, f32, vp]),
     "stx_amax": (i32, [vp, i64, vp, vp]),
     "stx_conv_weight_prep_batch": (i32, [C.POINTER(WprepJob), i32, vp]),
     "stx_conv2d_wgrad_plan": (i32, [C.POINTER(WgradParams), C.POINTER(sz)]),
@@ -185,6 +188,7 @@
     "stx_adam_ws": (sz, []),
     "stx_adam_step": (i32, [vp, vp, vp, vp, i64, f32, f32, f32, f32, vp, vp, vp]),
     "stx_adam_step_clear": (i32, [vp, vp, vp, vp, i64, f32, f32, f32, f32, vp, vp, vp, i32, vp]),
+    "stx_adam_step_prepared": (i32, [vp, vp, vp, vp, i64, f32, f32, f32, vp, vp, i32, vp]),
     "stx_instnorm_fwd": (i32, [vp, vp, vp, vp, vp, vp, vp, i32, i32, i32, f32, i32, vp, vp]),
     "stx_instnorm_bwd_ws": (sz, [i32, i32]),
     "stx_instnorm_param_grads": (i32, [C.POINTER(PGradJob), i32, vp]),
diff --git a/styletransfer_amd/csrc/conv16.hip b/styletransfer_amd/csrc/conv16.hip
--- a/styletransfer_amd/csrc/conv16.hip
+++ b/styletransfer_amd/csrc/conv16.hip
@@ -3,6 +3,7 @@
 
 #include "common.h"
 #include "conv_epi.h"
+#include "tail.h"
 #include "wprep.h"
 #include "../../include/stx.h"
 
@@ -1475,21 +1476,19 @@
 
 constexpr int WC_R = 16, WC_K = 64;
 
-__global__ void __launch_bounds__(256)
-weight_compose16_kernel(const float* __restrict__ A, int pitch, const float* __restrict__ a_amax,
-                        const float* __restrict__ W, const float* __restrict__ w_amax, int C,
-                        int cin, const float* __restrict__ scale, _Float16* __restrict__ slab,
-                        float* __restrict__ out_amax) {
+__device__ __forceinline__ void weight_compose16_body(
+    const float* __restrict__ A, int pitch, const float* __restrict__ a_amax,
+    const float* __restrict__ W, const float* __restrict__ w_amax, int C, int cin,
+    const float* __restrict__ scale, _Float16* __restrict__ slab, float* __restrict__ out_amax,
+    int bx, int by, float (*la)[WC_R], float (*lw)[WC_K]) {
   typedef _Float16 f16x4 __attribute__((ext_vector_type(4)));
   const int K = cin * 9;
-  __shared__ __attribute__((aligned(16))) float la[256][WC_R];
-  __shared__ __attribute__((aligned(16))) float lw[256][WC_K];
   float (*red)[WC_R * WC_K] = reinterpret_cast<float (*)[WC_R * WC_K]>(&lw[0][0]);
   const int tid = threadIdx.x, lane = tid & 63, wave = tid >> 6;
-  const int c0 = blockIdx.y * WC_R, k0 = blockIdx.x * WC_K;
+  const int c0 = by * WC_R, k0 = bx * WC_K;
   const float sc = scale ? *scale : 1.f;
   const float bound = fabsf(sc) * (float)C * read_amax(a_amax) * read_amax(w_amax);
-  if (blockIdx.x == 0 && blockIdx.y == 0 && tid < STX_AMAX_SLOTS) out_amax[tid] = bound;
+  if (bx == 0 && by == 0 && tid < STX_AMAX_SLOTS) out_amax[tid] = bound;
   const float sw = __builtin_ldexpf(1.f, 15 - amax_exp(bound));
   {
     constexpr int NLD = 256 * WC_K / 4 / 256;
@@ -1561,6 +1560,50 @@
     *reinterpret_cast<f16x4*>(slab + u0 * 8 + e0) = hi;
     *reinterpret_cast<f16x4*>(slab + u1 * 8 + e0) = lo;
   }
+}
+
+__global__ void __launch_bounds__(256)
+weight_compose16_kernel(const float* __restrict__ A, int pitch, const float* __restrict__ a_amax,
+                        const float* __restrict__ W, const float* __restrict__ w_amax, int C,
+                        int cin, const float* __restrict__ scale, _Float16* __restrict__ slab,
+                        float* __restrict__ out_amax) {
+  __shared__ __attribute__((aligned(16))) float la[256][WC_R];
+  __shared__ __attribute__((aligned(16))) float lw[256][WC_K];
+  weight_compose16_body(A, pitch, a_amax, W, w_amax, C, cin, scale, slab, out_amax, blockIdx.x,
+                        blockIdx.y, la, lw);
+}
+
+struct ComposeTail {
+  stx_loss_parts lp;
+  float* losses;
+  const float* extra;
+  float* total;
+  LossWF w;
+  int m;
+  int nblk, nbx;
+  int* step;
+  AdamScalars* sc;
+  double lr, b1, b2;
+};
+
+__global__ void __launch_bounds__(256)
+weight_compose16_tail_kernel(const float* __restrict__ A, int pitch,
+                             const float* __restrict__ a_amax, const float* __restrict__ W,
+                             const float* __restrict__ w_amax, int C, int cin,
+                             const float* __restrict__ scale, _Float16* __restrict__ slab,
+                             float* __restrict__ out_amax, ComposeTail t) {
+  __shared__ __attribute__((aligned(16))) float la[256][WC_R];
+  __shared__ __attribute__((aligned(16))) float lw[256][WC_K];
+  const int L = blockIdx.x;
+  if (L >= t.nblk) {
+    if (t.losses && L == t.nblk)
+      loss_finalize_body<4>(t.lp, t.losses, t.extra, t.m, t.w, t.total, &la[0][0]);
+    else if (threadIdx.x == 0)
+      adam_prepare_body(t.step, t.sc, t.lr, t.b1, t.b2);
+    return;
+  }
+  weight_compose16_body(A, pitch, a_amax, W, w_amax, C, cin, scale, slab, out_amax, L % t.nbx,
+                        L / t.nbx, la, lw);
 }
 
 static int launch16_unpool(const stx_conv_params& p, hipStream_t st) {
@@ -1765,6 +1808,59 @@
   return check_launch("stx_conv_weight_compose16");
 }
 
+extern "C" int stx_conv_weight_compose16_tail(
+    const float* A, int pitch, const float* a_amax, const float* w, const float* w_amax, int cout,
+    int cin, const float* scale, void* wtT16, float* out_amax, const stx_loss_parts* lp,
+    float* losses, const float* extra, int m, const float* w_host, float* total, int* step_dev,
+    void* adam_ws, float lr, float beta1, float beta2, void* stream) {
+  if (!A || !a_amax || !w || !w_amax || !wtT16 || !out_amax || cout <= 0 || cout > 256 ||
+      cin <= 0 || cin % 4 || pitch < cout || (reinterpret_cast<uintptr_t>(w) & 15)) {
+    set_error("stx_conv_weight_compose16_tail: invalid arguments (1 <= cout <= 256, "
+              "cin % 4 == 0, w 16-byte aligned)");
+    return STX_E_INVALID;
+  }
+  const long long total_h = (long long)rup(cout, 16) * 9 * 2 * rup(cin, 64);
+  if ((long long)cout * cin * 9 >= (1ll << 31) || total_h >= (1ll << 31)) {
+    set_error("stx_conv_weight_compose16_tail: weight too large");
+    return STX_E_INVALID;
+  }
+  if (lp && (lp->k < 0 || lp->k > 8 || m < 0 || lp->k + m > 16 || !losses || (m && !extra) ||
+             (total && !w_host))) {
+    set_error("stx_conv_weight_compose16_tail: invalid loss rider");
+    return STX_E_INVALID;
+  }
+  if (step_dev && !adam_ws) {
+    set_error("stx_conv_weight_compose16_tail: the prepare rider needs adam_ws");
+    return STX_E_INVALID;
+  }
+  hipStream_t st = (hipStream_t)stream;
+  if (cout % 16 || cin % 64)
+    (void)hipMemsetAsync(wtT16, 0, (size_t)total_h * sizeof(_Float16), st);
+  ComposeTail t{};
+  t.nbx = cdiv(cin * 9, WC_K);
+  t.nblk = t.nbx * cdiv(cout, WC_R);
+  if (lp) {
+    t.lp = *lp;
+    t.losses = losses;
+    t.extra = extra;
+    t.total = total;
+    t.m = m;
+    for (int i = 0; i < lp->k + m && w_host; ++i) t.w.w[i] = w_host[i];
+  }
+  if (step_dev) {
+    t.step = step_dev;
+    t.sc = (AdamScalars*)adam_ws;
+    t.lr = (double)lr;
+    t.b1 = (double)beta1;
+    t.b2 = (double)beta2;
+  }
+  const int riders = (lp ? 1 : 0) + (step_dev ? 1 : 0);
+  hipLaunchKernelGGL(weight_compose16_tail_kernel, dim3(t.nblk + riders), dim3(256), 0, st, A,
+                     pitch, a_amax, w, w_amax, cout, cin, scale,
+                     reinterpret_cast<_Float16*>(wtT16), out_amax, t);
+  return check_launch("stx_conv_weight_compose16_tail");
+}
+
 extern "C" int stx_conv_weight_prep16(const float* w, void* wt16, float* w_amax, int cout, int cin,
                                       int ks, int transpose, void* stream) {
   if (ks != 3 || !w || !wt16 || !w_amax || cout <= 0 || cin <= 0) {
diff --git a/styletransfer_amd/csrc/elementwise.hip b/styletransfer_amd/csrc/elementwise.hip
--- a/styletransfer_amd/csrc/elementwise.hip
+++ b/styletransfer_amd/csrc/elementwise.hip
@@ -1,4 +1,5 @@
 #include "common.h"
+#include "tail.h"
 #include "../../include/stx.h"
 
 namespace stx {
@@ -214,26 +215,19 @@
     dx[i] = y[i] > 0.f ? dy[i] : 0.f;
 }
 
-struct AdamScalars {
-  float step_size;
-  float bc2_sqrt;
-};
 
 __global__ void adam_prepare_kernel(int* step, AdamScalars* sc, double lr, double b1, double b2,
                                     float* clear, int clear_n) {
   for (int i = threadIdx.x; i < clear_n; i += blockDim.x) clear[i] = 0.f;
   if (threadIdx.x) return;
-  const int t = ++(*step);
-  const double bc1 = 1.0 - pow(b1, (double)t);
-  const double bc2 = 1.0 - pow(b2, (double)t);
-  sc->step_size = (float)(lr / bc1);
-  sc->bc2_sqrt = (float)sqrt(bc2);
+  adam_prepare_body(step, sc, lr, b1, b2);
 }
 
 __global__ void __launch_bounds__(256)
 adam_kernel(float* __restrict__ p, const float* __restrict__ g, float* __restrict__ m,
             float* __restrict__ v, long long n, float b1, float b2, float eps,
-            const AdamScalars* __restrict__ sc, int vec) {
+            const AdamScalars* __restrict__ sc, int vec, float* __restrict__ clear,
+            int clear_n) {
   const float step_size = sc->step_size, bc2s = sc->bc2_sqrt;
   const float w1 = 1.f - b1, w2 = 1.f - b2;
   const long long n4 = vec ? n / 4 : 0;
@@ -264,6 +258,8 @@
     const float denom = sqrtf(vv) / bc2s + eps;
     p[i] = p[i] + (-step_size * mm) / denom;
   }
+  if (blockIdx.x == gridDim.x - 1)
+    for (int i = threadIdx.x; i < clear_n; i += blockDim.x) clear[i] = 0.f;
 }
 
 __global__ void upsample_fwd_kernel(const float* __restrict__ x, float* __restrict__ y, int nc,
@@ -533,8 +529,23 @@
   const long long units = vec ? n / 4 : n;
   const int blocks = (int)std::max<long long>(1, std::min<long long>((units + 255) / 256, 4096));
   hipLaunchKernelGGL(adam_kernel, dim3(blocks), dim3(256), 0, st, p, g, m, v, n, beta1, beta2,
-                     eps, sc, vec);
+                     eps, sc, vec, (float*)nullptr, 0);
   return check_launch("stx_adam_step");
+}
+
+extern "C" int stx_adam_step_prepared(float* p, const float* g, float* m, float* v, long long n,
+                                      float beta1, float beta2, float eps, const void* ws,
+                                      float* clear, int clear_n, void* stream) {
+  if (n <= 0 || !p || !g || !m || !v || !ws || clear_n < 0 || (clear_n > 0 && !clear)) {
+    set_error("stx_adam_step_prepared: invalid args");
+    return STX_E_INVALID;
+  }
+  const int vec = (((uintptr_t)p | (uintptr_t)g | (uintptr_t)m | (uintptr_t)v) & 15) == 0;
+  const long long units = vec ? n / 4 : n;
+  const int blocks = (int)std::max<long long>(1, std::min<long long>((units + 255) / 256, 4096));
+  hipLaunchKernelGGL(adam_kernel, dim3(blocks), dim3(256), 0, (hipStream_t)stream, p, g, m, v, n,
+                     beta1, beta2, eps, (const AdamScalars*)ws, vec, clear, clear_n);
+  return check_launch("stx_adam_step_prepared");
 }
 
 extern "C" int stx_adam_step(float* p, const float* g, float* m, float* v, long long n, float lr,
diff --git a/styletransfer_amd/csrc/gram.hip b/styletransfer_amd/csrc/gram.hip
--- a/styletransfer_amd/csrc/gram.hip
+++ b/styletransfer_amd/csrc/gram.hip
@@ -1,4 +1,7 @@
+#include <type_traits>
+
 #include "common.h"
+#include "tail.h"
 #include "../../include/stx.h"
 
 namespace stx {
@@ -652,7 +655,7 @@
 __host__ __device__ inline int fin_groups(int nsplit) { return nsplit <= 8 ? 4 : nsplit <= 16 ? 2 : 1; }
 __host__ __device__ inline int fin_blocks_per_tile(int nsplit) { return FSUB / fin_groups(nsplit); }
 
-template <int G>
+template <int G, bool DEEP>
 __device__ __forceinline__ void gram_finalize_body_g(
     const float* __restrict__ ws, int c, int nsplit, float scale, float* __restrict__ g_out,
     const float* __restrict__ target, long long t_bstride, float* __restrict__ coef, int cpad,
@@ -672,6 +675,27 @@
     const f32x4* p4 = reinterpret_cast<const f32x4*>(src) + q4;
     constexpr int ST = GT * GT / 4;
     int k = kl;
+    auto rounds = [&](auto rc) {
+      constexpr int R = decltype(rc)::value;
+      f32x4 a[4 * R];
+#pragma unroll
+      for (int j = 0; j < 4 * R; ++j) a[j] = p4[(size_t)(k + j * KL) * ST];
+      __builtin_amdgcn_sched_barrier(0);
+#pragma unroll
+      for (int j = 0; j < R; ++j) {
+        s0 += a[4 * j + 0];
+        s1 += a[4 * j + 1];
+        s2 += a[4 * j + 2];
+        s3 += a[4 * j + 3];
+      }
+    };
+    if constexpr (DEEP && G == 1) {
+      for (; k + 15 * KL < nsplit; k += 16 * KL) rounds(std::integral_constant<int, 4>{});
+      if (k + 7 * KL < nsplit) {
+        rounds(std::integral_constant<int, 2>{});
+        k += 8 * KL;
+      }
+    }
     for (; k + 3 * KL < nsplit; k += 4 * KL) {
       const f32x4 a0 = p4[(size_t)(k + 0 * KL) * ST], a1 = p4[(size_t)(k + 1 * KL) * ST];
       const f32x4 a2 = p4[(size_t)(k + 2 * KL) * ST], a3 = p4[(size_t)(k + 3 * KL) * ST];
@@ -726,6 +750,7 @@
   }
 }
 
+template <bool DEEP>
 __device__ __forceinline__ void gram_finalize_body(const stx_gram_fin_job& q, int bx, int by) {
   __shared__ float part[FKL * (FEL + 1)];
   __shared__ float red[FNT / 64];
@@ -745,7 +770,7 @@
     }
   }
 #define STX_FIN_BODY(G)                                                                      \
-  gram_finalize_body_g<G>(q.parts, q.c, q.nsplit, q.scale, q.g_out, q.target, q.t_bstride,   \
+  gram_finalize_body_g<G, DEEP>(q.parts, q.c, q.nsplit, q.scale, q.g_out, q.target, q.t_bstride,   \
                           q.coef, q.cpad, q.cA, q.alpha, q.loss_parts, bx, by, part,         \
                           q.coef_amax)
   switch (fin_groups(q.nsplit)) {
@@ -756,8 +781,13 @@
 #undef STX_FIN_BODY
 }
 
+template <bool DEEP>
 __global__ void __launch_bounds__(FNT) gram_finalize_kernel(stx_gram_fin_job q) {
-  gram_finalize_body(q, blockIdx.x, blockIdx.y);
+  gram_finalize_body<DEEP>(q, blockIdx.x, blockIdx.y);
+}
+
+static bool fin_deep(int nsplit) {
+  return nsplit >= 16 * FKL && STX_KNOB("STX_FIN_DEEP", 1) != 0;
 }
 
 struct FinBatch {
@@ -766,26 +796,14 @@
   int njobs;
 };
 
+template <bool DEEP>
 __global__ void __launch_bounds__(FNT) gram_finalize_batch_kernel(FinBatch fb) {
   int j = 0;
   while (j + 1 < fb.njobs && (int)blockIdx.x >= fb.blk0[j + 1]) ++j;
   const stx_gram_fin_job& q = fb.job[j];
   const int local = blockIdx.x - fb.blk0[j];
   const int nt = cdiv(q.c, GT), nbx = nt * (nt + 1) / 2 * fin_blocks_per_tile(q.nsplit);
-  gram_finalize_body(q, local % nbx, local / nbx);
-}
-
-__device__ __forceinline__ float wave_sum_parts(const float* __restrict__ parts, int n, int lane) {
-  float s0 = 0.f, s1 = 0.f, s2 = 0.f, s3 = 0.f;
-  int i = lane;
-  for (; i + 192 < n; i += 256) {
-    s0 += parts[i];
-    s1 += parts[i + 64];
-    s2 += parts[i + 128];
-    s3 += parts[i + 192];
-  }
-  for (; i < n; i += 64) s0 += parts[i];
-  return wave_sum((s0 + s1) + (s2 + s3));
+  gram_finalize_body<DEEP>(q, local % nbx, local / nbx);
 }
 
 __global__ void sum_parts_kernel(const float* __restrict__ parts, int n, float inv,
@@ -799,10 +817,6 @@
        i += (long long)gridDim.x * blockDim.x)
     p[i] = 0.f;
 }
-
-struct LossWF {
-  float w[16];
-};
 
 static void gram_geometry(int c, int hw, int b, int& nsplit, int& split_len, int& ntu) {
   const int nt = cdiv(c, GT);
@@ -916,8 +930,11 @@
     return;
   }
   const int nt = cdiv(q.c, GT), ntu = nt * (nt + 1) / 2;
-  hipLaunchKernelGGL(gram_finalize_kernel, dim3(ntu * fin_blocks_per_tile(q.nsplit), q.b),
-                     dim3(FNT), 0, st, q);
+  const dim3 grid(ntu * fin_blocks_per_tile(q.nsplit), q.b);
+  if (fin_deep(q.nsplit))
+    hipLaunchKernelGGL(gram_finalize_kernel<true>, grid, dim3(FNT), 0, st, q);
+  else
+    hipLaunchKernelGGL(gram_finalize_kernel<false>, grid, dim3(FNT), 0, st, q);
   if (q.target && loss)
     hipLaunchKernelGGL(sum_parts_kernel, dim3(1), dim3(64), 0, st, q.loss_parts,
                        q.b * ntu * FSUB, (float)(1.0 / ((double)q.b * q.c * q.c)), loss);
@@ -940,21 +957,7 @@
                                                            int m, LossWF w,
                                                            float* __restrict__ total) {
   __shared__ float lv[8];
-  const int wave = threadIdx.x >> 6, lane = threadIdx.x & 63;
-  if (wave < lp.k) {
-    const float s = wave_sum_parts(lp.parts[wave], lp.nparts[wave], lane);
-    if (lane == 0) lv[wave] = s * lp.inv[wave];
-  }
-  __syncthreads();
-  if (threadIdx.x == 0) {
-    float t = 0.f;
-    for (int i = 0; i < lp.k; ++i) {
-      losses[i] = lv[i];
-      t += w.w[i] * lv[i];
-    }
-    for (int j = 0; j < m; ++j) t += w.w[lp.k + j] * extra[j];
-    if (total) *total = t;
-  }
+  loss_finalize_body<8>(lp, losses, extra, m, w, total, lv);
 }
 }
 
@@ -1088,7 +1091,7 @@
     return STX_E_INVALID;
   }
   FinBatch fb{};
-  int blocks = 0;
+  int blocks = 0, longest = 0;
   for (int j = 0; j < njobs; ++j) {
     const stx_gram_fin_job& q = jobs[j];
     if (!q.parts || q.c <= 0 || q.nsplit <= 0 || q.b <= 0 || !q.loss_parts) {
@@ -1098,12 +1101,17 @@
     const int nt = cdiv(q.c, GT);
     fb.job[j] = q;
     fb.blk0[j] = blocks;
+    longest = std::max(longest, q.nsplit);
     blocks += nt * (nt + 1) / 2 * fin_blocks_per_tile(q.nsplit) * q.b;
   }
   fb.blk0[njobs] = blocks;
   fb.njobs = njobs;
-  hipLaunchKernelGGL(gram_finalize_batch_kernel, dim3(blocks), dim3(FNT), 0, (hipStream_t)stream,
-                     fb);
+  if (fin_deep(longest))
+    hipLaunchKernelGGL(gram_finalize_batch_kernel<true>, dim3(blocks), dim3(FNT), 0,
+                       (hipStream_t)stream, fb);
+  else
+    hipLaunchKernelGGL(gram_finalize_batch_kernel<false>, dim3(blocks), dim3(FNT), 0,
+                       (hipStream_t)stream, fb);
   return check_launch("stx_gram_finalize_batch");
 }
 
diff --git a/styletransfer_amd/csrc/tail.h b/styletransfer_amd/csrc/tail.h
--- /dev/null
+++ b/styletransfer_amd/csrc/tail.h
@@ -0,0 +1,65 @@
+#ifndef STX_TAIL_H_
+#define STX_TAIL_H_
+
+#include "common.h"
+#include "../../include/stx.h"
+
+namespace stx {
+
+__device__ __forceinline__ float wave_sum_parts(const float* __restrict__ parts, int n, int lane) {
+  float s0 = 0.f, s1 = 0.f, s2 = 0.f, s3 = 0.f;
+  int i = lane;
+  for (; i + 192 < n; i += 256) {
+    s0 += parts[i];
+    s1 += parts[i + 64];
+    s2 += parts[i + 128];
+    s3 += parts[i + 192];
+  }
+  for (; i < n; i += 64) s0 += parts[i];
+  return wave_sum((s0 + s1) + (s2 + s3));
+}
+
+struct LossWF {
+  float w[16];
+};
+
+template <int NW>
+__device__ __forceinline__ void loss_finalize_body(const stx_loss_parts& lp,
+                                                   float* __restrict__ losses,
+                                                   const float* __restrict__ extra, int m,
+                                                   const LossWF& w, float* __restrict__ total,
+                                                   float* lv) {
+  const int wave = threadIdx.x >> 6, lane = threadIdx.x & 63;
+  for (int i = wave; i < lp.k; i += NW) {
+    const float s = wave_sum_parts(lp.parts[i], lp.nparts[i], lane);
+    if (lane == 0) lv[i] = s * lp.inv[i];
+  }
+  __syncthreads();
+  if (threadIdx.x == 0) {
+    float t = 0.f;
+    for (int i = 0; i < lp.k; ++i) {
+      losses[i] = lv[i];
+      t += w.w[i] * lv[i];
+    }
+    for (int j = 0; j < m; ++j) t += w.w[lp.k + j] * extra[j];
+    if (total) *total = t;
+  }
+}
+
+struct AdamScalars {
+  float step_size;
+  float bc2_sqrt;
+};
+
+__device__ __forceinline__ void adam_prepare_body(int* step, AdamScalars* sc, double lr,
+                                                  double b1, double b2) {
+  const int t = ++(*step);
+  const double bc1 = 1.0 - pow(b1, (double)t);
+  const double bc2 = 1.0 - pow(b2, (double)t);
+  sc->step_size = (float)(lr / bc1);
+  sc->bc2_sqrt = (float)sqrt(bc2);
+}
+
+}
+
+#endif
diff --git a/styletransfer_amd/ops.py b/styletransfer_amd/ops.py
--- a/styletransfer_amd/ops.py
+++ b/styletransfer_amd/ops.py
@@ -287,7 +287,7 @@
 
 
 def conv_weight_compose16(coef, coef_amax, w: torch.Tensor, w_amax, out_amax, scale=None,
-                          out=None):
+                          out=None, loss_job=None, adam_prepare=None):
     _req(w, "weight")
     _req(coef, "coef")
     cout, cin, ks, _ = w.shape
@@ -296,10 +296,26 @@
     if out is None:
         out = torch.empty(L.stx_conv_weight16_bytes(cin, cout, ks, 1), device=w.device,
                           dtype=torch.uint8)
-    check(L.stx_conv_weight_compose16(coef.data_ptr(), coef.shape[-1], coef_amax.data_ptr(),
-                                      w.data_ptr(), w_amax.data_ptr(), cout, cin, _p(scale),
-                                      out.data_ptr(), out_amax.data_ptr(), _stream()),
-          "stx_conv_weight_compose16")
+    if loss_job is None and adam_prepare is None:
+        check(L.stx_conv_weight_compose16(coef.data_ptr(), coef.shape[-1], coef_amax.data_ptr(),
+                                          w.data_ptr(), w_amax.data_ptr(), cout, cin, _p(scale),
+                                          out.data_ptr(), out_amax.data_ptr(), _stream()),
+              "stx_conv_weight_compose16")
+        return out
+    j, a = loss_job, adam_prepare
+    check(L.stx_conv_weight_compose16_tail(
+        coef.data_ptr(), coef.shape[-1], coef_amax.data_ptr(), w.data_ptr(), w_amax.data_ptr(),
+        cout, cin, _p(scale), out.data_ptr(), out_amax.data_ptr(),
+        C.byref(j.lp) if j else None, j.losses.data_ptr() if j else None,
+        _p(j.extra) if j else None, j.m if j else 0, j.w if j else None,
+        _p(j.total) if j else None,
+        a.step_dev.data_ptr() if a else None, a.ws.data_ptr() if a else None,
+        a.lr if a else 0.0, a.beta1 if a else 0.0, a.beta2 if a else 0.0, _stream()),
+        "stx_conv_weight_compose16_tail")
+    if j:
+        j.done = True
+    if a:
+        a.done = True
     return out
 
 
@@ -711,19 +727,32 @@
                        parts=gparts, nparts=nparts, mse_parts=mse_parts, mse_out=mse_out)
 
 
+class LossFinalizeJob:
+
+    def __init__(self, parts, losses, extra=None, weights=None, total=None):
+        self.lp = N.LossParts()
+        assert len(parts) <= 8
+        for i, (ptr, n, inv) in enumerate(parts):
+            self.lp.parts[i], self.lp.nparts[i], self.lp.inv[i] = ptr, n, inv
+        self.lp.k = len(parts)
+        self.losses, self.extra, self.total = losses, extra, total
+        self.m = 0 if extra is None else extra.numel()
+        self.w = None
+        if weights is not None:
+            self.w = (C.c_float * len(weights))(*[float(x) for x in weights])
+        self.done = False
+
+    def launch(self):
+        if not self.done:
+            check(lib().stx_loss_finalize(C.byref(self.lp), self.losses.data_ptr(),
+                                          _p(self.extra), self.m, self.w, _p(self.total),
+                                          _stream()), "stx_loss_finalize")
+            self.done = True
+        return self.losses
+
+
 def loss_finalize(parts, losses, extra=None, weights=None, total=None):
-    lp = N.LossParts()
-    assert len(parts) <= 8
-    for i, (ptr, n, inv) in enumerate(parts):
-        lp.parts[i], lp.nparts[i], lp.inv[i] = ptr, n, inv
-    lp.k = len(parts)
-    m = 0 if extra is None else extra.numel()
-    w = None
-    if weights is not None:
-        w = (C.c_float * len(weights))(*[float(x) for x in weights])
-    check(lib().stx_loss_finalize(C.byref(lp), losses.data_ptr(), _p(extra), m, w, _p(total),
-                                  _stream()), "stx_loss_finalize")
-    return losses
+    return LossFinalizeJob(parts, losses, extra, weights, total).launch()
 
 
 def gram_bwd_fused(coef, z, out=None, acc_scale=None, up_dp=None, aux=None, aux_scale=0.0,
@@ -892,6 +921,24 @@
     check(lib().stx_adam_step(p.data_ptr(), g.data_ptr(), m.data_ptr(), v.data_ptr(), p.numel(),
                               float(lr), float(beta1), float(beta2), float(eps),
                               step_dev.data_ptr(), ws.data_ptr(), _stream()), "stx_adam_step")
+
+
+class AdamPrepare:
+
+    def __init__(self, step_dev, ws, lr=1e-3, beta1=0.9, beta2=0.999):
+        self.step_dev, self.ws = step_dev, ws
+        self.lr, self.beta1, self.beta2 = float(lr), float(beta1), float(beta2)
+        self.done = False
+
+
+def adam_step_prepared(p, g, m, v, ws, beta1=0.9, beta2=0.999, eps=1e-8, clear=None):
+    if clear is not None:
+        _req(clear, "clear")
+    check(lib().stx_adam_step_prepared(p.data_ptr(), g.data_ptr(), m.data_ptr(), v.data_ptr(),
+                                       p.numel(), float(beta1), float(beta2), float(eps),
+                                       ws.data_ptr(), _p(clear),
+                                       0 if clear is None else clear.numel(), _stream()),
+          "stx_adam_step_prepared")
 
 
 def _mix_of(mix, n):
diff --git a/styletransfer_amd/vgg.py b/styletransfer_amd/vgg.py
--- a/styletransfer_amd/vgg.py
+++ b/styletransfer_amd/vgg.py
@@ -151,6 +151,7 @@
     grams: list = field(default_factory=lambda: [None] * 5)
     fin_jobs: list = None
     mse_parts: torch.Tensor = None
+    loss_job: object = None
 
 
 def tap_weights(style_weight, layer_weights=None):
@@ -176,7 +177,7 @@
 
 
 def loss_forward(feat: VGGFeatures, targets, x, c4, st: LossState | None = None,
-                 folded_weights=None, total=None, extra_slot=False):
+                 folded_weights=None, total=None, extra_slot=False, defer_loss=False):
     if st is None:
         st = LossState()
     dev = x.device
@@ -284,7 +285,11 @@
         if extra_slot:
             w += [0.0, 0.0, 1.0]
             extra = st.losses[5:9]
-    ops.loss_finalize(st.parts, st.losses[0:5], extra=extra, weights=w, total=total)
+    st.loss_job = ops.LossFinalizeJob(st.parts, st.losses[0:5], extra=extra, weights=w,
+                                      total=total)
+    if not defer_loss:
+        st.loss_job.launch()
+        st.loss_job = None
     return st
 
 
@@ -302,8 +307,14 @@
 
 
 def loss_backward(feat: VGGFeatures, st: LossState, g=None, dx=None, feature_grad=True,
-                  scratch=None):
+                  scratch=None, adam_prepare=None):
     z = st.z
+    job, st.loss_job = st.loss_job, None
+    if job is not None and N.knob("STX_TAIL_LOSS", "1") == "0":
+        job.launch()
+        job = None
+    if adam_prepare is not None and N.knob("STX_TAIL_ADAM", "1") == "0":
+        adam_prepare = None
     B = z[0].shape[0]
     sc = scratch if scratch is not None else {}
 
@@ -331,7 +342,7 @@
             N.knob("STX_COMPOSE", "1") != "0":
         sc["compose5"] = ops.conv_weight_compose16(
             st.coef[4], ca[4], feat.w[4], feat.wtT16[4][1], slot(am, COMPOSE_AMAX_SLOT),
-            scale=s(4), out=sc.get("compose5"))
+            scale=s(4), out=sc.get("compose5"), loss_job=job, adam_prepare=adam_prepare)
         cout, cin = VGG_CONV_SHAPES[4]
         if up4:
             dz4 = ops.conv2d(z[4], None, cout, cin, 3, out=buf("dz4", z[3].shape),
@@ -342,6 +353,8 @@
                              wt16=(sc["compose5"], slot(am, COMPOSE_AMAX_SLOT)),
                              in_amax=slot(am, 5))
     else:
+        if job is not None:
+            job.launch()
         dz5 = ops.gram_bwd_fused(st.coef[4], z[4], out=buf("dz5", z[4].shape), acc_scale=s(4),
                                  out_amax=slot(am, 6), z_amax=slot(am, 5) if sp else None)
         if up4:
@@ -440,13 +453,18 @@
 
     def _iteration(self):
         loss_forward(self.feat, self.targets, self.x, self.c4, self.st,
-                     folded_weights=(self.sw, self.cw), total=self.total)
+                     folded_weights=(self.sw, self.cw), total=self.total, defer_loss=True)
+        prep = ops.AdamPrepare(self.step_dev, self.adam_ws, self.lr, *self.betas)
         loss_backward(self.feat, self.st, dx=self.grad, feature_grad=False,
-                      scratch=self.scratch)
+                      scratch=self.scratch, adam_prepare=prep)
         if self.temporal is not None:
             _temporal_term(self)
-        ops.adam_step(self.x, self.grad, self.m, self.v, self.step_dev, self.adam_ws, self.lr,
-                      self.betas[0], self.betas[1], self.eps, clear=self.st.amax)
+        if prep.done:
+            ops.adam_step_prepared(self.x, self.grad, self.m, self.v, self.adam_ws,
+                                   self.betas[0], self.betas[1], self.eps, clear=self.st.amax)
+        else:
+            ops.adam_step(self.x, self.grad, self.m, self.v, self.step_dev, self.adam_ws,
+                          self.lr, self.betas[0], self.betas[1], self.eps, clear=self.st.amax)
         self.st.amax_cleared = True
 
     def retarget(self, content, init=None, temporal_ref=None, temporal_mask=None):
@@ -532,7 +550,7 @@
 
     def _closure(self):
         loss_forward(self.feat, self.targets, self.x, self.c4, self.st,
-                     folded_weights=(self.sw, self.cw), total=self.total)
+                     folded_weights=(self.sw, self.cw), total=self.total, defer_loss=True)
         loss_backward(self.feat, self.st, dx=self.grad, feature_grad=False,
                       scratch=self.scratch)
         if self.temporal is not None:
```
